# fgvieira/ngsLD

Hardware: AMD Instinct MI355X
Metric: SNP-pair EM-LD computations/sec @ n_ind=500 (higher is better)
Workload: dtype f64

## Files before the change

include/ngsld.h:

```cpp
#ifndef NGSLD_H
#define NGSLD_H

#include <stddef.h>
#include <stdint.h>

#ifdef __cplusplus
extern "C" {
#endif

typedef struct ngsld_ctx ngsld_ctx;

enum {
  NGSLD_OK = 0,
  NGSLD_ERR_INVALID = -1,
  NGSLD_ERR_DEVICE = -2,
  NGSLD_ERR_NOMEM = -3,
  NGSLD_ERR_NAN = -4,
  NGSLD_ERR_MAF_RANGE = -5,
  NGSLD_ERR_SINK = -6,
  NGSLD_ERR_UNSUPPORTED = -7
};

typedef struct {
  uint64_t max_kb_dist;
// ... 19 lines not shown
  uint32_t n_iter;
} ngsld_rec_ext;

typedef struct {
  uint32_t s1, s2_begin, count, reserved;
  uint64_t mask;
  uint64_t first_record;
} ngsld_item;

typedef struct {
  uint64_t s1_begin, s1_end;
  uint64_t n_pairs;
  uint64_t n_items;
  const ngsld_item *items;
  const ngsld_rec_std *std;
  const ngsld_rec_ext *ext;
  const char *text;
  uint64_t text_len;
} ngsld_batch;

typedef int (*ngsld_sink_fn)(void *user, const ngsld_batch *batch);

typedef int (*ngsld_read_sites_fn)(void *user, uint64_t site_begin, uint64_t n_sites, double *dst);

const char *ngsld_version(void);

int ngsld_create(int device, ngsld_ctx **ctx);
void ngsld_destroy(ngsld_ctx *ctx);
const char *ngsld_last_error(const ngsld_ctx *ctx);

int ngsld_set_geno_raw(ngsld_ctx *ctx, const double *gl_raw, uint64_t n_sites, uint64_t n_ind, int log_scale,
                       int ignore_miss_data, int on_device);
typedef struct {
  int32_t log_scale;
  int32_t ignore_miss_data;
  int32_t on_device;
  int32_t text_semantics;
  int32_t call_geno;
  int32_t per_individual_only;
  double N_thresh;
  double call_thresh;
} ngsld_geno_opts;
int ngsld_set_geno_raw_opts(ngsld_ctx *ctx, const double *gl_raw, uint64_t n_sites, uint64_t n_ind,
                            const ngsld_geno_opts *opts);
int ngsld_set_geno_lkl(ngsld_ctx *ctx, const double *geno_lkl, const double *maf, uint64_t n_sites, uint64_t n_ind,
                       int on_device);
int ngsld_get_maf(ngsld_ctx *ctx, double *maf_out);
int ngsld_set_pos_dist(ngsld_ctx *ctx, const double *pos_dist);

int ngsld_plan(ngsld_ctx *ctx, const ngsld_params *params, uint64_t *n_pairs);
int ngsld_plan_rows(ngsld_ctx *ctx, const uint64_t **row_off, const uint32_t **row_end);

int ngsld_run(ngsld_ctx *ctx, uint64_t s1_begin, uint64_t s1_end, ngsld_sink_fn sink, void *user);

int ngsld_set_text_output(ngsld_ctx *ctx, const char *const *labels, int enable);

int ngsld_reserve_text_buffers(ngsld_ctx *ctx, uint64_t bytes_per_row);

int ngsld_set_replay_source(ngsld_ctx *ctx, ngsld_read_sites_fn read, void *user);
int ngsld_set_replay_matrix(ngsld_ctx *ctx, const double *values);
int ngsld_set_replay(ngsld_ctx *ctx, int enable);
int ngsld_replay_stats(ngsld_ctx *ctx, uint64_t *pairs, uint64_t *sites);

int ngsld_set_exact_store(ngsld_ctx *ctx, int mode);
typedef struct {
  uint64_t pairs_flagged;
  uint64_t pairs_replayed;
  uint64_t pairs_on_device;
  uint64_t pairs_on_host;
  uint64_t sites_reevaluated;
  int32_t exact_store;
  int32_t text_rows_patched;
  double exact_store_build_s;
  uint64_t sites_degenerate;
} ngsld_replay_stats_t;
int ngsld_replay_info(ngsld_ctx *ctx, ngsld_replay_stats_t *out);

int ngsld_run_device(ngsld_ctx *ctx, uint64_t s1_begin, uint64_t s1_end, void *d_std, void *d_ext, void *hip_stream);
int ngsld_finish_device(ngsld_ctx *ctx);

int ngsld_last_kernel_time(ngsld_ctx *ctx, double *total_ms, uint64_t *n_launches, uint64_t *n_pairs);

const char *ngsld_pair_kernel(const ngsld_ctx *ctx);
int ngsld_describe_dispatch(uint64_t n_ind, int ignore_miss_data, char *buf, size_t buf_len);

int ngsld_set_tuning(ngsld_ctx *ctx, uint32_t pairs_per_item, uint64_t batch_pairs);

int ngsld_selftest(ngsld_ctx *ctx);

int ngsld_selftest_format(ngsld_ctx *ctx, uint64_t n, const ngsld_rec_std *std, const ngsld_rec_ext *ext, const double *dist,
                          const double *maf1, const double *maf2, char *text, uint64_t text_cap, uint64_t *row_len,
                          int32_t *needs_host);
int ngsld_selftest_printed(ngsld_ctx *ctx, uint64_t n, const double *x, int32_t precision, int32_t weight_type,
                           double min_weight, int64_t *micro, int32_t *micro_ok, int64_t *label, int32_t *label_rc);

typedef struct {
  uint64_t row_begin, row_end;
  uint64_t site_end;
} ngsld_slab;

int ngsld_window_ends(const double *pos_dist, uint64_t n_sites, const ngsld_params *params, uint32_t *row_end);

int ngsld_plan_slabs(const double *pos_dist, uint64_t n_sites, const ngsld_params *params, uint64_t max_slab_sites,
                     ngsld_slab *slabs, uint64_t cap, uint64_t *n_slabs);

uint64_t ngsld_slab_sites_for_budget(uint64_t n_ind, uint64_t budget_bytes);
uint64_t ngsld_sites_for_budget(uint64_t n_ind, uint64_t budget_bytes, int matrix_copies);

int ngsld_streamed_replay_info(ngsld_replay_stats_t *out);

int ngsld_set_memory_budget(int device, uint64_t bytes);

int ngsld_device_memory(int device, uint64_t *free_bytes, uint64_t *total_bytes);


int ngsld_run_streamed(int device, uint64_t n_sites, uint64_t n_ind, const double *pos_dist,
                       const ngsld_params *params, const ngsld_geno_opts *opts, uint64_t max_slab_sites,
                       ngsld_read_sites_fn read, void *read_user, double *maf_out, ngsld_sink_fn sink,
                       void *sink_user, uint64_t *n_pairs, uint64_t *n_slabs, char *err, size_t errlen);

int ngsld_run_streamed_text(int device, uint64_t n_sites, uint64_t n_ind, const double *pos_dist,
                            const ngsld_params *params, const ngsld_geno_opts *opts, uint64_t max_slab_sites,
                            ngsld_read_sites_fn read, void *read_user, double *maf_out, ngsld_sink_fn sink,
                            void *sink_user, uint64_t *n_pairs, uint64_t *n_slabs, char *err, size_t errlen,
                            const char *const *labels, int text_output);


int ngsld_plan_parts(const double *pos_dist, uint64_t n_sites, const ngsld_params *params, int n_parts, ngsld_slab *parts);

typedef int (*ngsld_multi_sink_fn)(void *user, int part, const ngsld_batch *batch);

int ngsld_run_multi(const int *devices, int n_devices, uint64_t n_sites, uint64_t n_ind, const double *pos_dist,
                    const ngsld_params *params, const ngsld_geno_opts *opts, const double *gl_raw,
                    ngsld_read_sites_fn read, void *read_user, double *maf_out, ngsld_multi_sink_fn sink, void *sink_user,
                    const char *const *labels, int text_output, uint64_t *pairs_per_part, char *err, size_t errlen);

enum { NGSLD_DIST_NONE = 0, NGSLD_DIST_UPLOAD = 1, NGSLD_DIST_PEER_COPY = 2, NGSLD_DIST_RCCL = 3 };
int ngsld_multi_last_distribution(void);

int ngsld_rccl_selftest(int device, uint64_t bytes, char *err, size_t errlen);

typedef struct {
  uint32_t struct_size;
  int32_t field;
  double max_kb_dist;
  double min_weight;
  int32_t weight_type;
  int32_t keep_heavy;
  int32_t precision;
  int32_t reserved;
  const char *const *subset;
  uint64_t n_subset;
} ngsld_prune_params;

typedef struct {
  uint32_t struct_size;
  uint32_t reserved;
  uint64_t pairs;
  uint64_t nodes, edges;
  uint64_t kept, excluded;
  uint64_t rounds;
  uint64_t host_nodes, host_edges, host_steps;
  double pairs_ms, edges_ms, graph_ms, rounds_ms, host_ms, total_ms;
} ngsld_prune_stats;

int ngsld_prune(ngsld_ctx *ctx, const ngsld_prune_params *params, const char *const *labels, uint8_t *site_state,
// ... 75 lines not shown
```

ngsld_amd/capi.py:

```python
from __future__ import annotations

import ctypes as C
import os
import subprocess

import numpy as np

PKG_DIR = os.path.dirname(os.path.abspath(__file__))
REPO_DIR = os.path.dirname(PKG_DIR)
LIB_PATH = os.environ.get("NGSLD_LIB") or os.path.join(PKG_DIR, "libngsld.so")
CLI_PATH = os.path.join(PKG_DIR, "bin", "ngsLD")

OK, ERR_INVALID, ERR_DEVICE, ERR_NOMEM, ERR_NAN, ERR_MAF_RANGE, ERR_SINK, ERR_UNSUPPORTED = 0, -1, -2, -3, -4, -5, -6, -7


class Params(C.Structure):
    _fields_ = [("max_kb_dist", C.c_uint64), ("max_snp_dist", C.c_uint64), ("min_maf", C.c_double),
                ("ignore_miss_data", C.c_int32), ("extend_out", C.c_int32), ("rnd_sample", C.c_double),
                ("seed", C.c_uint64), ("first_row", C.c_uint64)]


class GenoOpts(C.Structure):
    _fields_ = [("log_scale", C.c_int32), ("ignore_miss_data", C.c_int32), ("on_device", C.c_int32),
                ("text_semantics", C.c_int32), ("call_geno", C.c_int32), ("per_individual_only", C.c_int32),
                ("N_thresh", C.c_double), ("call_thresh", C.c_double)]


REC_STD = np.dtype([("r2_ExpG", "<f8"), ("D", "<f8"), ("Dp", "<f8"), ("r2", "<f8")])
REC_EXT = np.dtype([("hap", "<f8", (4,)), ("n_ind_data", "<u4"), ("n_iter", "<u4")])


ITEM = np.dtype([("s1", "<u4"), ("s2_begin", "<u4"), ("count", "<u4"), ("reserved", "<u4"), ("mask", "<u8"),
                 ("first_record", "<u8")])


class Batch(C.Structure):
    _fields_ = [("s1_begin", C.c_uint64), ("s1_end", C.c_uint64), ("n_pairs", C.c_uint64), ("n_items", C.c_uint64),
                ("items", C.c_void_p), ("std", C.c_void_p), ("ext", C.c_void_p), ("text", C.c_void_p),
                ("text_len", C.c_uint64)]


def items_to_pairs(items: np.ndarray) -> tuple[np.ndarray, np.ndarray]:
    if len(items) == 0:
        return np.zeros(0, dtype=np.uint64), np.zeros(0, dtype=np.uint64)
    bits = (items["mask"][:, None] >> np.arange(64, dtype=np.uint64)[None, :]) & np.uint64(1)
    bits &= (np.arange(64)[None, :] < items["count"][:, None]).astype(np.uint64)
    idx, c = np.nonzero(bits)
    return items["s1"][idx].astype(np.uint64), (items["s2_begin"][idx].astype(np.uint64) + c.astype(np.uint64))


def items_from_pairs(s1: np.ndarray, s2: np.ndarray, span: int = 64) -> np.ndarray:
    s1, s2 = np.asarray(s1, dtype=np.int64), np.asarray(s2, dtype=np.int64)
    chunk = (s2 - s1 - 1) // span
    key = s1 * (1 << 32) + chunk
    uniq, first, inv = np.unique(key, return_index=True, return_inverse=True)
    items = np.zeros(len(uniq), dtype=ITEM)
    items["s1"] = s1[first]
    items["s2_begin"] = s1[first] + 1 + chunk[first] * span
    items["first_record"] = first
    np.bitwise_or.at(items["mask"], inv, np.uint64(1) << (s2 - items["s2_begin"][inv]).astype(np.uint64))
    last = np.zeros(len(uniq), dtype=np.int64)
    np.maximum.at(last, inv, s2 - items["s2_begin"][inv].astype(np.int64))
    items["count"] = last + 1
    return items


SINK_FN = C.CFUNCTYPE(C.c_int, C.c_void_p, C.POINTER(Batch))
MULTI_SINK_FN = C.CFUNCTYPE(C.c_int, C.c_void_p, C.c_int, C.POINTER(Batch))
READ_FN = C.CFUNCTYPE(C.c_int, C.c_void_p, C.c_uint64, C.c_uint64, C.c_void_p)
SLAB = np.dtype([("row_begin", "<u8"), ("row_end", "<u8"), ("site_end", "<u8")])

SYMBOLS = [
    "ngsld_version", "ngsld_create", "ngsld_destroy", "ngsld_last_error", "ngsld_set_geno_raw",
    "ngsld_set_geno_raw_opts", "ngsld_set_geno_lkl",
    "ngsld_get_maf", "ngsld_set_pos_dist", "ngsld_plan", "ngsld_plan_rows", "ngsld_run", "ngsld_run_device", "ngsld_set_text_output",
    "ngsld_set_replay_source", "ngsld_set_replay_matrix", "ngsld_set_replay", "ngsld_replay_stats", "ngsld_finish_device",
    "ngsld_set_exact_store", "ngsld_replay_info",
    "ngsld_plan_parts", "ngsld_run_multi", "ngsld_multi_last_distribution", "ngsld_rccl_selftest",
    "ngsld_last_kernel_time", "ngsld_pair_kernel", "ngsld_describe_dispatch", "ngsld_set_tuning", "ngsld_selftest", "ngsld_selftest_format",
    "ngsld_selftest_printed", "ngsld_reserve_text_buffers",
    "ngsld_window_ends", "ngsld_plan_slabs", "ngsld_slab_sites_for_budget", "ngsld_sites_for_budget", "ngsld_streamed_replay_info", "ngsld_set_memory_budget", "ngsld_device_memory", "ngsld_run_streamed", "ngsld_run_streamed_text",
    "ngsld_host_read_geno_bin_range",
    "ngsld_host_set_threads", "ngsld_host_read_pos", "ngsld_host_pos_dist", "ngsld_host_label", "ngsld_host_free_pos", "ngsld_host_pos_slice",
    "ngsld_host_geno_size_ok", "ngsld_host_read_geno_bin", "ngsld_host_read_geno_text", "ngsld_host_format_header", "ngsld_host_format_pair",
    "ngsld_host_format_double", "ngsld_host_write_batch", "ngsld_host_replay_pair", "ngsld_host_missing_call_log",
    "ngsld_host_gz_open", "ngsld_host_gz_close",
    "ngsld_prune", "ngsld_host_prune_graph", "ngsld_host_prune_label",
    "ngsld_decay", "ngsld_decay_bins", "ngsld_host_decay_fit",
    "ngsld_blocks", "ngsld_blocks_sites", "ngsld_blocks_matrix", "ngsld_blocks_text",
    "ngsld_site_ld", "ngsld_site_ld_get",
]


class ReplayStats(C.Structure):
    _fields_ = [("pairs_flagged", C.c_uint64), ("pairs_replayed", C.c_uint64), ("pairs_on_device", C.c_uint64),
                ("pairs_on_host", C.c_uint64), ("sites_reevaluated", C.c_uint64), ("exact_store", C.c_int32),
                ("text_rows_patched", C.c_int32), ("exact_store_build_s", C.c_double), ("sites_degenerate", C.c_uint64)]


class PruneParams(C.Structure):
    _fields_ = [("struct_size", C.c_uint32), ("field", C.c_int32), ("max_kb_dist", C.c_double), ("min_weight", C.c_double),
                ("weight_type", C.c_int32), ("keep_heavy", C.c_int32), ("precision", C.c_int32), ("reserved", C.c_int32),
                ("subset", C.POINTER(C.c_char_p)), ("n_subset", C.c_uint64)]


class PruneStats(C.Structure):
    _fields_ = [("struct_size", C.c_uint32), ("reserved", C.c_uint32), ("pairs", C.c_uint64), ("nodes", C.c_uint64),
                ("edges", C.c_uint64), ("kept", C.c_uint64), ("excluded", C.c_uint64), ("rounds", C.c_uint64),
                ("host_nodes", C.c_uint64), ("host_edges", C.c_uint64), ("host_steps", C.c_uint64),
                ("pairs_ms", C.c_double), ("edges_ms", C.c_double), ("graph_ms", C.c_double), ("rounds_ms", C.c_double),
                ("host_ms", C.c_double), ("total_ms", C.c_double)]


class DecayParams(C.Structure):
    _fields_ = [("struct_size", C.c_uint32), ("fields", C.c_uint32), ("bin_size", C.c_double), ("max_kb_dist", C.c_double),
                ("min_maf", C.c_double)]


class DecayStats(C.Structure):
    _fields_ = [("struct_size", C.c_uint32), ("lds", C.c_uint32), ("pairs", C.c_uint64), ("pairs_counted", C.c_uint64),
                ("bins", C.c_uint64), ("bin_slots", C.c_uint64), ("chunks", C.c_uint64), ("pairs_ms", C.c_double),
                ("bin_ms", C.c_double), ("total_ms", C.c_double)]


class BlocksParams(C.Structure):
    _fields_ = [("struct_size", C.c_uint32), ("fields", C.c_uint32), ("chr", C.c_char_p), ("start", C.c_uint64),
                ("end", C.c_uint64)]


class BlocksStats(C.Structure):
    _fields_ = [("struct_size", C.c_uint32), ("reserved", C.c_uint32), ("members", C.c_uint64), ("sites", C.c_uint64),
                ("pairs", C.c_uint64), ("pairs_in_region", C.c_uint64), ("cells_na", C.c_uint64), ("host_rows", C.c_uint64),
                ("chunks", C.c_uint64), ("pairs_ms", C.c_double), ("scatter_ms", C.c_double), ("format_ms", C.c_double),
                ("total_ms", C.c_double)]


class SiteLdParams(C.Structure):
    _fields_ = [("struct_size", C.c_uint32), ("fields", C.c_uint32), ("max_kb_dist", C.c_double), ("min_maf", C.c_double),
                ("linked_min", C.c_double), ("abs_value", C.c_int32), ("reserved", C.c_int32)]


class SiteLdStats(C.Structure):
    _fields_ = [("struct_size", C.c_uint32), ("lds", C.c_uint32), ("pairs", C.c_uint64), ("pairs_counted", C.c_uint64),
                ("sites_with_pairs", C.c_uint64), ("chunks", C.c_uint64), ("pairs_ms", C.c_double), ("site_ms", C.c_double),
                ("total_ms", C.c_double)]


TEXT_FN = C.CFUNCTYPE(C.c_int, C.c_void_p, C.c_void_p, C.c_uint64)


class DecayFitResult(C.Structure):
    _fields_ = [("rate", C.c_double), ("ld_max", C.c_double), ("ld_min", C.c_double), ("sse", C.c_double),
                ("n_bins", C.c_uint64)]


DECAY_FIELDS = ("r2_ExpG", "D", "Dp", "r2")


class NgsldError(RuntimeError):
    def __init__(self, code: int, msg: str):
        super().__init__(f"ngsld error {code}: {msg}")
        self.code = code
        self.msg = msg


def build(force: bool = False, jobs: int = 8) -> None:
    csrc = os.path.join(PKG_DIR, "csrc")
    if force:
        subprocess.check_call(["make", "-s", "-C", csrc, "clean"])
    subprocess.check_call(["make", "-s", f"-j{jobs}", "-C", csrc, "all"])


_lib = None


def lib() -> C.CDLL:
    global _lib
    if _lib is None:
        if not os.path.exists(LIB_PATH):
            raise FileNotFoundError(f"{LIB_PATH} is missing: run ngsld_amd.capi.build() (or make -C ngsld_amd/csrc); "
                                    "there is no fallback implementation")
        L = C.CDLL(LIB_PATH)
        vp, u64, dbl = C.c_void_p, C.c_uint64, C.c_double
        L.ngsld_version.restype = C.c_char_p
        L.ngsld_create.argtypes = [C.c_int, C.POINTER(vp)]
        L.ngsld_destroy.argtypes = [vp]
        L.ngsld_destroy.restype = None
        L.ngsld_last_error.argtypes = [vp]
        L.ngsld_last_error.restype = C.c_char_p
        L.ngsld_set_geno_raw.argtypes = [vp, vp, u64, u64, C.c_int, C.c_int, C.c_int]
        L.ngsld_set_geno_raw_opts.argtypes = [vp, vp, u64, u64, C.POINTER(GenoOpts)]
        L.ngsld_set_geno_lkl.argtypes = [vp, vp, vp, u64, u64, C.c_int]
        L.ngsld_get_maf.argtypes = [vp, vp]
        L.ngsld_set_pos_dist.argtypes = [vp, vp]
        L.ngsld_plan.argtypes = [vp, C.POINTER(Params), C.POINTER(u64)]
        L.ngsld_plan_rows.argtypes = [vp, C.POINTER(C.POINTER(C.c_uint64)), C.POINTER(C.POINTER(C.c_uint32))]
        L.ngsld_run.argtypes = [vp, u64, u64, SINK_FN, vp]
        L.ngsld_run_device.argtypes = [vp, u64, u64, vp, vp, vp]
        if hasattr(L, "ngsld_set_replay_source"):
            L.ngsld_set_replay_source.argtypes = [vp, READ_FN, vp]
            if hasattr(L, "ngsld_set_replay_matrix"):
                L.ngsld_set_replay_matrix.argtypes = [vp, vp]
            L.ngsld_set_replay.argtypes = [vp, C.c_int]
            L.ngsld_replay_stats.argtypes = [vp, C.POINTER(u64), C.POINTER(u64)]
        if hasattr(L, "ngsld_replay_info"):
            L.ngsld_set_exact_store.argtypes = [vp, C.c_int]
            L.ngsld_replay_info.argtypes = [vp, C.POINTER(ReplayStats)]
            L.ngsld_finish_device.argtypes = [vp]
        if hasattr(L, "ngsld_set_text_output"):
            L.ngsld_set_text_output.argtypes = [vp, C.POINTER(C.c_char_p), C.c_int]
        L.ngsld_last_kernel_time.argtypes = [vp, C.POINTER(dbl), C.POINTER(u64), C.POINTER(u64)]
        L.ngsld_set_tuning.argtypes = [vp, C.c_uint32, u64]
        if hasattr(L, "ngsld_pair_kernel"):
            L.ngsld_pair_kernel.argtypes = [vp]
            L.ngsld_pair_kernel.restype = C.c_char_p
        L.ngsld_selftest.argtypes = [vp]
        if hasattr(L, "ngsld_selftest_format"):
            L.ngsld_selftest_format.argtypes = [vp, u64, vp, vp, vp, vp, vp, C.c_char_p, u64, vp, C.POINTER(C.c_int32)]
            L.ngsld_selftest_printed.argtypes = [vp, u64, vp, C.c_int32, C.c_int32, dbl, vp, vp, vp, vp]
        L.ngsld_window_ends.argtypes = [vp, u64, C.POINTER(Params), vp]
        L.ngsld_plan_slabs.argtypes = [vp, u64, C.POINTER(Params), u64, vp, u64, C.POINTER(u64)]
        L.ngsld_slab_sites_for_budget.argtypes = [u64, u64]
        L.ngsld_slab_sites_for_budget.restype = u64
        if hasattr(L, "ngsld_sites_for_budget"):
            L.ngsld_sites_for_budget.argtypes = [u64, u64, C.c_int]
            L.ngsld_sites_for_budget.restype = u64
        L.ngsld_device_memory.argtypes = [C.c_int, C.POINTER(u64), C.POINTER(u64)]
        L.ngsld_run_streamed.argtypes = [C.c_int, u64, u64, vp, C.POINTER(Params), C.POINTER(GenoOpts), u64, READ_FN, vp,
                                         vp, SINK_FN, vp, C.POINTER(u64), C.POINTER(u64), C.c_char_p, C.c_size_t]
        if hasattr(L, "ngsld_run_multi"):
            L.ngsld_plan_parts.argtypes = [vp, u64, C.POINTER(Params), C.c_int, vp]
            L.ngsld_run_multi.argtypes = [C.POINTER(C.c_int), C.c_int, u64, u64, vp, C.POINTER(Params), C.POINTER(GenoOpts),
                                          vp, READ_FN, vp, vp, MULTI_SINK_FN, vp, C.POINTER(C.c_char_p), C.c_int,
                                          C.POINTER(u64), C.c_char_p, C.c_size_t]
        if hasattr(L, "ngsld_multi_last_distribution"):
            L.ngsld_multi_last_distribution.argtypes = []
        if hasattr(L, "ngsld_rccl_selftest"):
            L.ngsld_rccl_selftest.argtypes = [C.c_int, u64, C.c_char_p, C.c_size_t]
        L.ngsld_host_read_geno_bin_range.argtypes = [C.c_char_p, u64, u64, u64, vp, C.c_char_p, C.c_size_t]
        L.ngsld_host_set_threads.argtypes = [C.c_int]
        L.ngsld_host_set_threads.restype = None
        L.ngsld_host_read_pos.argtypes = [C.c_char_p, C.c_int, u64, C.POINTER(vp), C.c_char_p, C.c_size_t]
        L.ngsld_host_pos_dist.argtypes = [vp]
        L.ngsld_host_pos_dist.restype = C.POINTER(dbl)
        L.ngsld_host_label.argtypes = [vp, u64]
        L.ngsld_host_label.restype = C.c_char_p
        L.ngsld_host_free_pos.argtypes = [vp]
        L.ngsld_host_free_pos.restype = None
        L.ngsld_host_pos_slice.argtypes = [vp, u64, u64]
        L.ngsld_host_pos_slice.restype = vp
        L.ngsld_host_geno_size_ok.argtypes = [u64, u64, u64]
        L.ngsld_host_read_geno_bin.argtypes = [C.c_char_p, u64, u64, vp, C.c_char_p, C.c_size_t]
        L.ngsld_host_read_geno_text.argtypes = [C.c_char_p, C.c_int, C.c_int, u64, u64, vp, C.POINTER(C.c_int),
                                                C.c_char_p, C.c_size_t]
        L.ngsld_host_format_header.argtypes = [C.c_char_p, C.c_size_t, C.c_int]
        L.ngsld_host_format_header.restype = C.c_size_t
        L.ngsld_host_format_pair.argtypes = [C.c_char_p, C.c_size_t, C.c_char_p, C.c_char_p, dbl, vp, vp, dbl, dbl]
        L.ngsld_host_format_pair.restype = C.c_size_t
        L.ngsld_host_format_double.argtypes = [C.c_char_p, C.c_size_t, dbl, C.c_int]
        L.ngsld_host_format_double.restype = C.c_size_t
        L.ngsld_host_write_batch.argtypes = [C.POINTER(Batch), vp, vp, vp, C.c_int, C.c_int]
        L.ngsld_host_replay_pair.argtypes = [vp, vp, u64, C.POINTER(GenoOpts), vp, vp, vp]
        if hasattr(L, "ngsld_host_gz_open"):
            L.ngsld_host_gz_open.argtypes = [C.c_char_p, C.c_int, C.POINTER(vp), C.POINTER(C.c_int)]
            L.ngsld_host_gz_close.argtypes = [vp]
        if hasattr(L, "ngsld_prune"):
            L.ngsld_prune.argtypes = [vp, C.POINTER(PruneParams), C.POINTER(C.c_char_p), vp, C.POINTER(PruneStats)]
            L.ngsld_host_prune_graph.argtypes = [u64, vp, u64, vp, vp, vp, C.c_int, vp, C.POINTER(u64)]
            L.ngsld_host_prune_label.argtypes = [dbl, C.c_int, C.c_char, C.POINTER(C.c_int64)]
        if hasattr(L, "ngsld_decay"):
            L.ngsld_decay.argtypes = [vp, C.POINTER(DecayParams), C.POINTER(DecayStats)]
            L.ngsld_decay_bins.argtypes = [vp, u64, vp, vp, vp, C.POINTER(u64)]
            L.ngsld_host_decay_fit.argtypes = [u64, vp, vp, C.c_int, dbl, dbl, C.POINTER(DecayFitResult)]
        if hasattr(L, "ngsld_blocks"):
            L.ngsld_blocks.argtypes = [vp, C.POINTER(BlocksParams), C.POINTER(C.c_char_p), C.POINTER(BlocksStats)]
            L.ngsld_blocks_sites.argtypes = [vp, u64, vp, C.POINTER(u64)]
            L.ngsld_blocks_matrix.argtypes = [vp, C.c_int, vp, vp]
            L.ngsld_blocks_text.argtypes = [vp, C.c_int, TEXT_FN, vp, C.POINTER(BlocksStats)]
        if hasattr(L, "ngsld_site_ld"):
            L.ngsld_site_ld.argtypes = [vp, C.POINTER(SiteLdParams), C.POINTER(SiteLdStats)]
            L.ngsld_site_ld_get.argtypes = [vp, C.c_int, vp, vp, vp, vp, vp]
        _lib = L
    return _lib


def prune_label(x: float, prec: int = 4, weight_type: str = "a") -> int | None:
    out = C.c_int64()
    rc = lib().ngsld_host_prune_label(float(x), prec, weight_type.encode(), C.byref(out))
    if rc == ERR_INVALID:
        return None
    if rc != OK:
        raise NgsldError(rc, "label out of range")
    return out.value


# ... 546 lines not shown
                    exts.append(np.frombuffer(C.string_at(b.ext, n * REC_EXT.itemsize), dtype=REC_EXT).copy())
            items = np.frombuffer(C.string_at(b.items, b.n_items * ITEM.itemsize), dtype=ITEM) if b.n_items else \
                np.zeros(0, dtype=ITEM)
            a, bb = items_to_pairs(items)
            assert len(a) == n
            if len(items):
                assert np.array_equal(items["first_record"], np.concatenate([[0], np.cumsum(
                    [bin(int(m)).count("1") for m in items["mask"]])[:-1]]).astype(np.uint64))
            s1s.append(a)
            s2s.append(bb)
            return 0

        cb = SINK_FN(sink)
        self._check(self._L.ngsld_run(self._h, s1_begin, s1_end, cb, None))
        cat = lambda xs, dt: np.concatenate(xs) if xs else np.zeros(0, dtype=dt)
        return (cat(s1s, np.uint64), cat(s2s, np.uint64), cat(stds, REC_STD),
                cat(exts, REC_EXT) if self.extend_out else None)

    def run_to_fd(self, s1_begin: int, s1_end: int, fd: int, pos_handle, pos_dist: np.ndarray | None, maf: np.ndarray,
                  n_threads: int) -> int:
        maf = np.ascontiguousarray(maf, dtype=np.float64)
        pd_ptr = None if pos_dist is None else np.ascontiguousarray(pos_dist, dtype=np.float64).ctypes.data
        total, rc_box = [0], [0]

        libc = C.CDLL(None, use_errno=True)
        libc.write.argtypes = [C.c_int, C.c_void_p, C.c_size_t]
        libc.write.restype = C.c_ssize_t

        def sink(_user, bp):
            b = bp.contents
            total[0] += b.n_pairs
            if b.text:
                off = 0
                while off < b.text_len:
                    w = libc.write(fd, b.text + off, min(b.text_len - off, 1 << 30))
                    if w <= 0:
                        return 1
                    off += w
                return 0
            rc_box[0] = self._L.ngsld_host_write_batch(bp, pos_handle, pd_ptr, maf.ctypes.data, n_threads, fd)
            return 0 if rc_box[0] == OK else 1

        self._check(self._L.ngsld_run(self._h, s1_begin, s1_end, SINK_FN(sink), None))
        return total[0]

    def set_text_output(self, labels: list[str] | None, enable: bool = True) -> None:
        arr = None
        if labels is not None:
            arr = (C.c_char_p * len(labels))(*[l.encode() for l in labels])
        self._check(self._L.ngsld_set_text_output(self._h, arr, int(enable)))

    def run_text(self, s1_begin: int = 0, s1_end: int | None = None) -> tuple[bytes, int]:
        s1_end = self.n_sites if s1_end is None else s1_end
        parts, fallbacks = [], [0]

        def sink(_user, bp):
            b = bp.contents
            if b.text:
                parts.append(C.string_at(b.text, b.text_len))
            else:
                fallbacks[0] += 1
            return 0

        self._check(self._L.ngsld_run(self._h, s1_begin, s1_end, SINK_FN(sink), None))
        return b"".join(parts), fallbacks[0]

    def run_discard(self, s1_begin: int = 0, s1_end: int | None = None) -> int:
        s1_end = self.n_sites if s1_end is None else s1_end
        total = [0]

        def sink(_user, bp):
            total[0] += bp.contents.n_pairs
            return 0

        self._check(self._L.ngsld_run(self._h, s1_begin, s1_end, SINK_FN(sink), None))
        return total[0]

    def run_device(self, s1_begin: int, s1_end: int, d_std: int, d_ext: int | None, stream: int | None = None) -> None:
        self._check(self._L.ngsld_run_device(self._h, s1_begin, s1_end, d_std, d_ext, stream))

    def pair_kernel(self) -> str:
        return self._L.ngsld_pair_kernel(self._h).decode()

    def last_kernel_time(self) -> tuple[float, int, int]:
        ms, nl, npairs = C.c_double(), C.c_uint64(), C.c_uint64()
        self._check(self._L.ngsld_last_kernel_time(self._h, C.byref(ms), C.byref(nl), C.byref(npairs)))
        return ms.value, nl.value, npairs.value

    def prune(self, labels: list[str] | None, field: int = 7, max_kb_dist: float = float("inf"), min_weight: float = 0.0,
              weight_type: str = "a", keep_heavy: bool = False, subset: list[str] | None = None,
              precision: int = 4) -> tuple[np.ndarray, dict]:
        arr = None if labels is None else (C.c_char_p * len(labels))(*[l.encode() for l in labels])
        sub = None if subset is None else (C.c_char_p * max(len(subset), 1))(*[l.encode() for l in subset])
        p = PruneParams(C.sizeof(PruneParams), field, float(max_kb_dist), float(min_weight), ord(weight_type), int(keep_heavy),
                        precision, 0, sub, 0 if subset is None else len(subset))
        st = PruneStats()
        st.struct_size = C.sizeof(PruneStats)
        state = np.zeros(max(self.n_sites, 1), dtype=np.uint8)
        self._check(self._L.ngsld_prune(self._h, C.byref(p), arr, state.ctypes.data, C.byref(st)))
        return state[:self.n_sites], {k: getattr(st, k) for k, _ in PruneStats._fields_ if k not in ("struct_size", "reserved")}

    def decay(self, ld=("r2",), bin_size: float = 250, max_kb_dist: float = float("inf"),
              min_maf: float = 0.0) -> tuple[dict, dict]:
        ld = (ld,) if isinstance(ld, str) else tuple(ld)
        bad = [f for f in ld if f not in DECAY_FIELDS]
        if bad or not ld:
            raise ValueError(f"ld must name some of {DECAY_FIELDS}: {bad}")
        mask = sum(1 << DECAY_FIELDS.index(f) for f in set(ld))
        names = [f for k, f in enumerate(DECAY_FIELDS) if (mask >> k) & 1]
        p = DecayParams(C.sizeof(DecayParams), mask, float(bin_size), float(max_kb_dist), float(min_maf))
        st = DecayStats()
        st.struct_size = C.sizeof(DecayStats)
        self._check(self._L.ngsld_decay(self._h, C.byref(p), C.byref(st)))
        nb = st.bins
        dist = np.zeros(max(nb, 1))
        cnt = np.zeros(max(nb, 1), dtype=np.uint64)
        mean = np.zeros((max(nb, 1), len(names)))
        got = C.c_uint64()
        self._check(self._L.ngsld_decay_bins(self._h, nb, dist.ctypes.data, cnt.ctypes.data, mean.ctypes.data, C.byref(got)))
        assert got.value == nb
        bins = {"dist": dist[:nb], "n": cnt[:nb]}
        for k, f in enumerate(names):
            bins[f] = mean[:nb, k].copy()
        return bins, {k: getattr(st, k) for k, _ in DecayStats._fields_ if k != "struct_size"}

    def site_ld(self, ld=("r2",), max_kb_dist: float = float("inf"), min_maf: float = 0.0, linked_min: float = 0.5,
                abs_value: bool = True) -> tuple[dict, dict]:
        ld = (ld,) if isinstance(ld, str) else tuple(ld)
        bad = [f for f in ld if f not in DECAY_FIELDS]
        if bad or not ld:
            raise ValueError(f"ld must name some of {DECAY_FIELDS}: {bad}")
        mask = sum(1 << DECAY_FIELDS.index(f) for f in set(ld))
        p = SiteLdParams(C.sizeof(SiteLdParams), mask, float(max_kb_dist), float(min_maf), float(linked_min), int(bool(abs_value)), 0)
        st = SiteLdStats()
        st.struct_size = C.sizeof(SiteLdStats)
        self._check(self._L.ngsld_site_ld(self._h, C.byref(p), C.byref(st)))
        m = max(self.n_sites, 1)
        sites = {"n": np.zeros(m, dtype=np.uint64)}
        for k, f in enumerate(DECAY_FIELDS):
            if not (mask >> k) & 1:
                continue
            sites[f"sum_{f}"], sites[f"max_{f}"] = np.zeros(m, dtype=np.int64), np.zeros(m, dtype=np.int64)
            sites[f"linked_{f}"], sites[f"mean_{f}"] = np.zeros(m, dtype=np.uint64), np.zeros(m)
            self._check(self._L.ngsld_site_ld_get(self._h, 4 + k, sites["n"].ctypes.data, sites[f"sum_{f}"].ctypes.data,
                                                  sites[f"max_{f}"].ctypes.data, sites[f"linked_{f}"].ctypes.data,
                                                  sites[f"mean_{f}"].ctypes.data))
        sites = {k: v[:self.n_sites] for k, v in sites.items()}
        return sites, {k: getattr(st, k) for k, _ in SiteLdStats._fields_ if k != "struct_size"}

    def blocks(self, labels: list[str], chr: str, start: int, end: int,
               ld=("r2", "Dp")) -> tuple[np.ndarray, dict, dict]:
        ld = (ld,) if isinstance(ld, str) else tuple(ld)
        bad = [f for f in ld if f not in DECAY_FIELDS]
        if bad or not ld:
            raise ValueError(f"ld must name some of {DECAY_FIELDS}: {bad}")
        mask = sum(1 << DECAY_FIELDS.index(f) for f in set(ld))
        arr = (C.c_char_p * max(len(labels), 1))(*[l.encode() for l in labels]) if labels is not None else None
        p = BlocksParams(C.sizeof(BlocksParams), mask, chr.encode(), int(start), int(end))
        st = BlocksStats()
        st.struct_size = C.sizeof(BlocksStats)
        self._check(self._L.ngsld_blocks(self._h, C.byref(p), arr, C.byref(st)))
        m = st.sites
        sites = np.zeros(max(m, 1), dtype=np.uint64)
        got = C.c_uint64()
        self._check(self._L.ngsld_blocks_sites(self._h, m, sites.ctypes.data, C.byref(got)))
        assert got.value == m
# ... 26 lines not shown
```

ngsld_amd/csrc/cli_main.cpp:

```cpp
#include <getopt.h>
#include <zlib.h>
#include <sys/stat.h>
#include <sys/mman.h>
#include <unistd.h>

#include <cmath>
#include <cstdio>
#include <cstdlib>
#include <cstring>
#include <ctime>
#include <memory>
#include <string>
#include <algorithm>
#include <chrono>
#include <thread>
#include <vector>

#include "../../include/ngsld.h"
#include "../../include/ngsld_host.h"
#include "knobs.h"
#include "host_buf.h"

namespace {

// ... 1096 lines not shown
    if (site_begin + n > r->n_sites) return 1;
    memcpy(dst, r->raw + site_begin * r->n_ind * 3, n * r->n_ind * 3 * sizeof(double));
    return 0;
  };
  if (ngsld::test_knob_is("REPLAY_SOURCE", "0"))
    raw.reset();
  else if (ngsld::test_knob_is("REPLAY_SOURCE", "callback")) {
    if (ngsld_set_replay_source(ctx, read_raw, &raw_src) != NGSLD_OK) error("ngsld_set_replay_source", ngsld_last_error(ctx));
  } else if (ngsld_set_replay_matrix(ctx, raw.get()) != NGSLD_OK)
    error("ngsld_set_replay_matrix", ngsld_last_error(ctx));

  if (pars.verbose >= 1) fprintf(stderr, "==> Getting sites coordinates\n");
  ngsld_pos *pos = nullptr;
  if (pars.in_pos) {
    if (early.pos_done) {
      if (early.pos_rc != NGSLD_OK) error(pos_error_function(early.pos_err, pars.in_pos), early.pos_err);
      pos = early.pos;
    } else if (ngsld_host_read_pos(pars.in_pos, pars.in_pos_header ? 1 : 0, pars.n_sites, &pos, err, sizeof(err)) != NGSLD_OK)
      error(pos_error_function(err, pars.in_pos), err);
    if (pars.verbose >= 6)
      for (uint64_t s = 0; s < (pars.n_sites < 10 ? pars.n_sites : 10); s++)
        fprintf(stderr, "%lu\t%f\n", (unsigned long)s, ngsld_host_pos_dist(pos)[s]);
  }
  if (ngsld_set_pos_dist(ctx, pos ? ngsld_host_pos_dist(pos) : nullptr) != NGSLD_OK)
    error("ngsld_set_pos_dist", ngsld_last_error(ctx));

  if (pars.verbose >= 1) fprintf(stderr, "==> Launching threads...\n");
  ngsld_params lp;
  lp.max_kb_dist = pars.max_kb_dist;
  lp.max_snp_dist = pars.max_snp_dist;
  lp.min_maf = pars.min_maf;
  lp.ignore_miss_data = pars.ignore_miss_data ? 1 : 0;
  lp.extend_out = pars.extend_out ? 1 : 0;
  lp.rnd_sample = pars.rnd_sample;
  lp.seed = pars.seed;
  lp.first_row = 0;
  uint64_t n_pairs = 0;
  timing_report.mark("positions");
  if (ngsld_plan(ctx, &lp, &n_pairs) != NGSLD_OK) error("ngsld_plan", ngsld_last_error(ctx));
  std::vector<double> maf(pars.n_sites);
  if (ngsld_get_maf(ctx, maf.data()) != NGSLD_OK) error("ngsld_get_maf", ngsld_last_error(ctx));
  timing_report.mark("plan");
  if (write_tsv && !host_text_only()) {
    std::vector<const char *> lab;
    if (pos) {
      lab.resize(pars.n_sites);
      for (uint64_t s = 0; s < pars.n_sites; s++) lab[s] = ngsld_host_label(pos, s);
    }
    if (ngsld_set_text_output(ctx, pos ? lab.data() : nullptr, 1) != NGSLD_OK)
      error("ngsld_set_text_output", ngsld_last_error(ctx));
  }
  if (pars.verbose >= 1) fprintf(stderr, "==> Waiting for all threads to finish...\n");
  SinkState sink;
  sink.pars = &pars;
  sink.pos = pos;
  sink.pos_dist = pos ? ngsld_host_pos_dist(pos) : nullptr;
  sink.maf = &maf;
  timing_report.mark("labels to the device");
  rc = write_tsv ? ngsld_run(ctx, 0, pars.n_sites, write_batch, &sink) : NGSLD_OK;
  timing_report.mark("pair kernels + text + write");
  if (rc == NGSLD_ERR_MAF_RANGE) error("haplo_freq", ngsld_last_error(ctx));
  if (rc != NGSLD_OK) error("ngsld_run", ngsld_last_error(ctx));
  if (prune.given) {
    run_prune(ctx, pars, prune, pos);
    timing_report.mark("pruning");
  }
  if (decay.given) {
    run_decay(ctx, pars, decay);
    timing_report.mark("LD decay");
  }
  if (blocks.given) {
    run_blocks(ctx, pars, blocks, pos);
    timing_report.mark("LD blocks");
  }
  if (site.given) {
    run_site(ctx, pars, site, pos);
    timing_report.mark("site LD");
  }
  if (write_tsv && pars.verbose >= 2) {
    ngsld_replay_stats_t st{};
    (void)ngsld_replay_info(ctx, &st);
    fprintf(stderr, "==> %lu of %lu pairs replayed in the reference's operation order (%lu on the device, %lu on host threads)\n",
            (unsigned long)st.pairs_replayed, (unsigned long)n_pairs, (unsigned long)st.pairs_on_device, (unsigned long)st.pairs_on_host);
  }

  if (pars.verbose >= 1) fprintf(stderr, "==> Freeing memory...\n");
  close_output(pars.out_fh);
  ngsld_host_free_pos(pos);
  ngsld_destroy(ctx);
  timing_report.mark("free");
  if (pars.verbose >= 1) fprintf(stderr, "Done!\n");
  return 0;
}
```

ngsld_amd/csrc/engine.h:

```cpp
#pragma once

#include "knobs.h"

#include <hip/hip_runtime.h>
#include <sched.h>
#include <dlfcn.h>
#include <sys/mman.h>

#include <algorithm>
#include <atomic>
#include <chrono>
#include <cmath>
#include <condition_variable>
#include <functional>
#include <cstdio>
#include <cstdlib>
#include <cstring>
#include <limits>
#include <mutex>
#include <new>
#include <string>
#include <thread>
#include <unordered_map>
#include <vector>
// ... 141 lines not shown
    while ((int)threads_.size() < T - 1) {
      const int id = (int)threads_.size() + 1;
      threads_.emplace_back([this, id] { loop(id); });
    }
    {
      std::lock_guard<std::mutex> lk(mu_);
      job_ = [&fn](int t) { fn(t); };
      n_ = T;
      left_ = T - 1;
      ++epoch_;
    }
    cv_.notify_all();
    fn(0);
    std::unique_lock<std::mutex> lk(mu_);
    done_.wait(lk, [this] { return left_ == 0; });
    job_ = nullptr;
  }

 private:
  void loop(int id) {
    uint64_t seen = 0;
    for (;;) {
      std::function<void(int)> job;
      {
        std::unique_lock<std::mutex> lk(mu_);
        cv_.wait(lk, [&] { return stop_ || epoch_ != seen; });
        if (stop_) return;
        seen = epoch_;
        if (id >= n_) continue;
        job = job_;
      }
      job(id);
      std::lock_guard<std::mutex> lk(mu_);
      if (--left_ == 0) done_.notify_all();
    }
  }
  std::vector<std::thread> threads_;
  std::mutex mu_;
  std::condition_variable cv_, done_;
  std::function<void(int)> job_;
  int n_ = 0, left_ = 0;
  uint64_t epoch_ = 0;
  bool stop_ = false;
};

}
}

using namespace ngsld;
using namespace ngsld::eng;

struct FlagRow {
  uint64_t rec, off;
  uint32_t len, s1, s2, pad;
};
constexpr uint32_t kFlagRowsCap = 1024;

struct ngsld_ctx {
  int device = 0;
  hipStream_t stream = nullptr, stream2 = nullptr, copy_stream = nullptr;
  hipStream_t text_stream = nullptr;
  hipEvent_t ev_scan_done[3] = {nullptr, nullptr, nullptr};
  std::string err;

  uint64_t n_sites = 0, n_ind = 0;
  uint32_t np = 0;
  PairConfig cfg{};
  bool have_geno = false;
  DevBuf<double> d_planes, d_maf, d_mean, d_rsx, d_sc4;
  DevBuf<int> d_status;
  std::vector<double> h_maf, h_pos_dist;
  DevBuf<uint64_t> d_hard_masks;
  DevBuf<double> d_hard_u;
  DevBuf<int> d_all_hard, d_odd_missing;
  int h_odd_missing = 0;
  bool missing_canonical = false;
  int h_all_hard = 0, h_prep_status = 0;
  uint32_t mask_words = 0;
  DevBuf<uint8_t> d_skip;
  DevBuf<uint32_t> d_skip_count;
  uint32_t h_skip_count = 0;
  bool skip_on = true;
  bool skip_kernels = false;

  bool planned = false;
  ngsld_params params{};
  std::vector<uint64_t> h_row_off, h_item_off;
  std::vector<uint32_t> h_row_end;
  std::vector<uint8_t> h_keep;
  std::vector<Item> h_items;
  std::vector<uint64_t> h_run_off;
  uint64_t run_len = 0;
  std::vector<uint64_t> run_ends;
  int n_cus = 256;
  DevBuf<Run> d_runs;
  DevBuf<uint64_t> d_row_off, d_item_off, d_row_seed, d_row_count;
  DevBuf<uint32_t> d_row_end;
  DevBuf<uint8_t> d_keep;
  DevBuf<Item> d_items;
  uint64_t n_items = 0;

  int kernel_choice = kChooseAuto;
  uint32_t pairs_per_item = 16;
  uint64_t batch_pairs = 1ull << 23;
  bool batch_pairs_set = false;

  static constexpr int kSlots = 3;
  DevBuf<ngsld_rec_std> d_std[kSlots];
  DevBuf<ngsld_rec_ext> d_ext[kSlots];
  PinBuf<ngsld_rec_std> h_std[kSlots];
  PinBuf<ngsld_rec_ext> h_ext[kSlots];
  hipEvent_t ev_kernel_done[kSlots] = {nullptr, nullptr, nullptr}, ev_copy_done[kSlots] = {nullptr, nullptr, nullptr};
  bool run_direct = true, run_taper = true;
  int run_streams = 1;
  bool timed_overlap = false;

  bool text_mode = false, have_labels = false;
  uint64_t max_label = 6;
  DevBuf<char> d_labels, d_text[kSlots], d_scan_tmp, d_scan_tmp_b;
  DevBuf<uint64_t> d_label_off, d_lens[kSlots], d_offs[kSlots], d_text_meta[kSlots];
  DevBuf<double> d_cum;
  DevBuf<uint32_t> d_infc;
  PinBuf<char> h_text[kSlots];
  PinBuf<uint64_t> h_text_meta[kSlots];
  std::thread reserve_thread;

  bool replay_on = true;
  ngsld_read_sites_fn replay_read = nullptr;
  void *replay_user = nullptr;
  const double *replay_matrix = nullptr;
  std::mutex replay_mu;
  hipStream_t replay_stream = nullptr;
  std::mutex replay_stream_mu;
  ngsld_geno_opts gopts{};
  bool normalised = false;
  DevBuf<uint32_t> d_flags[kSlots], d_flags_dev;
  PinBuf<uint32_t> h_flags[kSlots], h_flags_dev;
  PinBuf<uint32_t> h_flag_bits;
  PinBuf<FlagRow> h_flag_rows[kSlots];
  uint32_t flag_cap[kSlots] = {0, 0, 0}, flag_cap_dev = 0;
  bool replay_device = true;
  uint64_t replayed_on_device = 0;
  uint64_t text_rows_patched = 0;
  DevBuf<double> d_xplanes, d_xmaf;
  DevBuf<double> d_xT;
  std::atomic<bool> xT_ready{false};
  DevBuf<uint32_t> d_xperm;
  DevBuf<uint32_t> d_xdepth;
  struct LaneScratch {
    DevBuf<ReplayEntry> list;
    DevBuf<uint64_t> keys_a, keys_b;
    DevBuf<uint32_t> vals_a, vals_b;
    DevBuf<char> temp;
    void release() { list.release(); keys_a.release(); keys_b.release(); vals_a.release(); vals_b.release(); temp.release(); }
  } lane_scratch[kSlots], lane_scratch_dev;
  PinBuf<double> h_xstage[2];
  std::thread exact_thread;
  std::atomic<int> exact_state{0};
  std::atomic<uint64_t> exact_frontier{0};
  std::atomic<bool> exact_cancel{false};
  std::mutex exact_mu;
  std::condition_variable exact_cv;
  int exact_rc = 0;
  std::string exact_msg;
  hipStream_t exact_stream = nullptr;
  ReplayPool exact_pool;
// ... 145 lines not shown
  EventPair() = default;
  EventPair(const EventPair &) = delete;
  EventPair &operator=(const EventPair &) = delete;
  ~EventPair() {
    if (a) (void)hipEventDestroy(a);
    if (b) (void)hipEventDestroy(b);
  }
  hipError_t create() {
    hipError_t e = hipEventCreate(&a);
    return e == hipSuccess ? hipEventCreate(&b) : e;
  }
  hipError_t add_elapsed(double *ms) const {
    float t = 0.f;
    const hipError_t e = hipEventElapsedTime(&t, a, b);
    if (e == hipSuccess) *ms += t;
    return e;
  }
};

int launch_record_items(ngsld_ctx *c, EventPair &ev, uint64_t r0, uint64_t r1, double *ms, uint64_t *chunks,
                        const std::function<void(const ngsld_item *items, uint64_t n_items)> &launch);

inline unsigned blocks_for(uint64_t threads, unsigned per_block = 256) { return (unsigned)((threads + per_block - 1) / per_block); }
inline double ms_since(std::chrono::steady_clock::time_point t0) {
  return std::chrono::duration<double, std::milli>(std::chrono::steady_clock::now() - t0).count();
}
template <class P, class S>
int check_struct_sizes(ngsld_ctx *c, const P *p, const char *p_name, const S *stats, const char *s_name) {
  if (p == nullptr || p->struct_size != sizeof(P))
    return fail(c, NGSLD_ERR_INVALID, std::string(p_name) + ": struct_size must be sizeof(" + p_name + ")");
  if (stats != nullptr && stats->struct_size < sizeof(uint32_t)) return fail(c, NGSLD_ERR_INVALID, std::string(s_name) + ": struct_size not set");
  return NGSLD_OK;
}
template <class S>
void copy_stats(S *out, const S &s) {
  if (out == nullptr) return;
  const uint32_t want = out->struct_size;
  std::memcpy(out, &s, std::min<size_t>(want, sizeof(S)));
  out->struct_size = want;
}
inline int field_list(uint32_t mask, int field[4]) {
  int ns = 0;
  for (int f = 0; f < 4; ++f)
    if ((mask >> f) & 1u) field[ns++] = f;
  return ns;
}

int send_flag_rows(ngsld_ctx *c, const uint32_t *d_flags, uint32_t cap, bool dev_applied, const uint64_t *d_offs, const uint64_t *d_lens,
                   uint64_t n_records, uint64_t base, FlagRow *h_rows, hipStream_t st);
int replay_pairs_on_host(ngsld_ctx *c, const uint32_t *s1, const uint32_t *s2, size_t n, ngsld_rec_std *out_std, ngsld_rec_ext *out_ext);
unsigned usable_threads();
hipStream_t replay_stream_of(ngsld_ctx *c);
int ensure_host_items(ngsld_ctx *c);
int fetch_replay_site(ngsld_ctx *c, uint64_t s, std::vector<double> &tmp, ReplaySite *out);
int flagged_records(ngsld_ctx *c, const uint32_t *h_head, const uint32_t *d_flags, uint32_t cap, uint64_t n,
                    std::vector<uint64_t> &recs, bool dev_applied = false);
bool room_for(uint64_t need_bytes, uint64_t device_margin, uint64_t budget_margin);
bool lkl_device_eligible(const ngsld_ctx *c);
bool exact_store_is_free(const ngsld_ctx *c);
inline bool exact_store_started(const ngsld_ctx *c) { return c->exact_state.load() >= 1; }
int start_exact_store(ngsld_ctx *c);
int reserve_device_run(ngsld_ctx *c, uint64_t n_records);
int wait_exact_store(ngsld_ctx *c, uint64_t need_sites, bool *have);
int ensure_exact_store(ngsld_ctx *c);
void stop_exact_store(ngsld_ctx *c);
inline uint64_t exact_sites_needed(const ngsld_ctx *c, uint64_t r0, uint64_t r1) {
  uint64_t need = r1;
  for (uint64_t r = r0; r < r1 && r < c->h_row_end.size(); ++r) need = std::max<uint64_t>(need, c->h_row_end[r]);
  return std::min<uint64_t>(need, c->n_sites);
}
bool exact_store_wanted(const ngsld_ctx *c, uint64_t pending);
int try_device_replay_lkl(ngsld_ctx *c, uint32_t *d_flags, uint32_t cap, uint64_t out_base, uint64_t n, ngsld_rec_std *d_std,
                          ngsld_rec_ext *d_ext, hipStream_t st, bool flag_text, int slot, bool *applied, uint64_t need_sites);
int device_replay_lkl(ngsld_ctx *c, uint32_t *d_flags, uint32_t cap, uint64_t out_base, uint64_t n, ngsld_rec_std *d_std,
                      ngsld_rec_ext *d_ext, hipStream_t st, bool flag_text, int slot);
int replay_flagged(ngsld_ctx *c, const std::vector<uint64_t> &recs, uint64_t base, ngsld_rec_std *h_std,
                   ngsld_rec_ext *h_ext, ngsld_rec_std *d_std, ngsld_rec_ext *d_ext, hipStream_t st,
                   std::vector<uint32_t> *sites1 = nullptr, std::vector<uint32_t> *sites2 = nullptr);
int reset_flags(ngsld_ctx *c, DevBuf<uint32_t> &buf, uint64_t n, uint32_t cap, hipStream_t stream);
int send_flag_head(ngsld_ctx *c, const uint32_t *d_flags, uint32_t *h_head, uint32_t cap, hipStream_t st, bool with_list = true);
int device_replay(ngsld_ctx *c, uint32_t *d_flags, uint32_t cap, uint64_t out_base, uint64_t n, ngsld_rec_std *d_std,
                  ngsld_rec_ext *d_ext, hipStream_t st, int slot);
int finish_device_run(ngsld_ctx *c);

}
}
```

ngsld_amd/csrc/engine.hip:

```cpp
#include "engine.h"

#include <atomic>

namespace ngsld {
namespace eng {

thread_local std::string g_create_error;

int set_geno_common(ngsld_ctx *c, const double *gl, const double *maf, uint64_t n_sites, uint64_t n_ind,
                    const ngsld_geno_opts &o, bool normalised) {
  if (c == nullptr) return NGSLD_ERR_INVALID;
  const int log_scale = o.log_scale, ignore_miss = o.ignore_miss_data, on_device = o.on_device;
  Range range_("ngsld:set_geno (upload + per-site prep)");
  if (o.call_geno && o.N_thresh > o.call_thresh)
    return fail(c, NGSLD_ERR_INVALID, "missing data threshold must be smaller than calling genotype threshold!");
  if (gl == nullptr || n_sites == 0 || n_ind == 0) return fail(c, NGSLD_ERR_INVALID, "empty genotype matrix");
  if (normalised && maf == nullptr) return fail(c, NGSLD_ERR_INVALID, "maf missing");
  if (n_sites >= 0xffffffffull) return fail(c, NGSLD_ERR_UNSUPPORTED, "n_sites must be below 2^32 - 1");
  PairConfig cfg;
  if (!pair_config(n_ind, &cfg, c->kernel_choice, ignore_miss != 0))
    return fail(c, NGSLD_ERR_UNSUPPORTED, "n_ind is outside the supported range");
  HIP_TRY(c, hipSetDevice(c->device));
  (void)hipGetLastError();
  {
// ... 58 lines not shown
    const char *pe = test_knob("PREP_EXACT");
    a.exact_chain = (pe != nullptr && std::strcmp(pe, "0") != 0) ? 1 : 0;
  }
  a.N_thresh = o.N_thresh;
  a.call_thresh = o.call_thresh;
  a.maf = c->d_maf.p;
  a.mean_e = c->d_mean.p;
  a.rsx = c->d_rsx.p;
  a.status = c->d_status.p;
  c->missing_canonical = false;
  const bool look_for_odd_missing = o.text_semantics && log_scale && !o.call_geno && !normalised;
  if (look_for_odd_missing) {
    HIP_TRY(c, c->d_odd_missing.resize(1));
    HIP_TRY(c, hipMemsetAsync(c->d_odd_missing.p, 0, sizeof(int), c->stream));
    a.odd_missing = c->d_odd_missing.p;
    a.missing_canon = replay_missing_raw_text();
  }
  if (on_device) {
    a.raw = gl;
    a.maf_in = maf;
    a.site0 = 0;
    a.n_sites = n_sites;
    HIP_TRY(c, launch_prep(a, c->stream));
  } else {
    const uint64_t site_bytes = n_ind * 3 * sizeof(double);
    uint64_t stage_bytes = 64ull << 20;
    if (const char *e = test_knob("STAGE_BYTES")) stage_bytes = std::strtoull(e, nullptr, 10);
    uint64_t chunk = stage_bytes / site_bytes;
    if (chunk < 1) chunk = 1;
    if (chunk > n_sites) chunk = n_sites;
    DevBuf<double> stage[2], maf_stage[2];
    hipEvent_t prepped[2] = {nullptr, nullptr};
    for (int k = 0; k < 2; ++k) {
      HIP_TRY(c, stage[k].resize(chunk * n_ind * 3));
      if (normalised) HIP_TRY(c, maf_stage[k].resize(chunk));
      HIP_TRY(c, hipEventCreateWithFlags(&prepped[k], hipEventDisableTiming));
    }
    int rc = NGSLD_OK;
    uint64_t k = 0;
    if (trace) std::fprintf(stderr, "[trace] set_geno: device buffers + staging allocated at %.2f ms\n", ms_since());
    for (uint64_t s0 = 0; s0 < n_sites && rc == NGSLD_OK; s0 += chunk, ++k) {
      const int b = (int)(k & 1);
      const uint64_t m = std::min(chunk, n_sites - s0);
      hipError_t e = hipSuccess;
      if (k >= 2) e = hipEventSynchronize(prepped[b]);
      if (e == hipSuccess)
        e = hipMemcpyAsync(stage[b].p, gl + s0 * n_ind * 3, m * site_bytes, hipMemcpyHostToDevice, c->copy_stream);
      if (e == hipSuccess && normalised)
        e = hipMemcpyAsync(maf_stage[b].p, maf + s0, m * sizeof(double), hipMemcpyHostToDevice, c->copy_stream);
      if (e == hipSuccess) e = hipStreamSynchronize(c->copy_stream);
      if (trace) std::fprintf(stderr, "[trace] set_geno: chunk %llu (%llu sites) on the device at %.2f ms\n", (unsigned long long)k, (unsigned long long)m, ms_since());
      a.raw = stage[b].p;
      a.maf_in = normalised ? maf_stage[b].p : nullptr;
      a.site0 = s0;
      a.n_sites = m;
      if (e == hipSuccess) e = launch_prep(a, c->stream);
      if (e == hipSuccess) e = hipEventRecord(prepped[b], c->stream);
      if (e != hipSuccess) rc = hip_fail(c, e, "chunked genotype upload");
    }
    hipError_t e = hipStreamSynchronize(c->stream);
    if (trace) std::fprintf(stderr, "[trace] set_geno: last prep kernel done at %.2f ms\n", ms_since());
    for (int q = 0; q < 2; ++q) {
      stage[q].release();
      maf_stage[q].release();
      if (prepped[q]) (void)hipEventDestroy(prepped[q]);
    }
    if (trace) std::fprintf(stderr, "[trace] set_geno: staging buffers freed at %.2f ms\n", ms_since());
    if (rc != NGSLD_OK) return rc;
    if (e != hipSuccess) return hip_fail(c, e, "chunked genotype upload");
  }
  c->h_skip_count = 0;
  const bool look_for_skip = c->skip_on && c->replay_on && c->replay_device && c->exact_mode != 0;
  c->skip_kernels = cfg.kernel == kRun || (cfg.kernel == kMulti && cfg.form == 0 && cfg.waves == 2);
  if (look_for_skip) {
    HIP_TRY(c, c->d_skip.resize(n_sites));
    HIP_TRY(c, c->d_skip_count.resize(1));
    HIP_TRY(c, hipMemsetAsync(c->d_skip_count.p, 0, sizeof(uint32_t), c->stream));
    HIP_TRY(c, launch_site_skip(c->d_planes.p, 3ull * c->np, c->np, (uint32_t)n_ind, ignore_miss, c->d_maf.p, n_sites, c->d_skip.p,
                                c->d_skip_count.p, c->stream));
    HIP_TRY(c, hipMemcpyAsync(&c->h_skip_count, c->d_skip_count.p, sizeof(uint32_t), hipMemcpyDeviceToHost, c->stream));
  } else {
    c->d_skip.release();
  }
  HIP_TRY(c, launch_pack_scalars(c->d_maf.p, c->d_mean.p, c->d_rsx.p, c->d_skip.p, c->d_sc4.p, n_sites, c->stream));
  int &all_hard = c->h_all_hard;
  all_hard = 0;
  const char *hk = test_knob("HARD_KERNEL");
  const bool try_hard = n_ind <= kHardMaxInd && !o.per_individual_only && !(hk != nullptr && std::strcmp(hk, "0") == 0);
  if (try_hard) {
    c->mask_words = (uint32_t)((n_ind + 63) / 64);
    HIP_TRY(c, c->d_hard_masks.resize((size_t)n_sites * 4 * c->mask_words));
    HIP_TRY(c, c->d_hard_u.resize(n_sites));
    HIP_TRY(c, c->d_all_hard.resize(1));
    all_hard = 1;
    HIP_TRY(c, hipMemcpyAsync(c->d_all_hard.p, &all_hard, sizeof(int), hipMemcpyHostToDevice, c->stream));
    HIP_TRY(c, launch_classify_hard(c->d_planes.p, 3ull * c->np, c->np, (uint32_t)n_ind, n_sites, c->d_hard_masks.p,
                                    c->d_hard_u.p, c->d_all_hard.p, c->stream));
    HIP_TRY(c, hipMemcpyAsync(&all_hard, c->d_all_hard.p, sizeof(int), hipMemcpyDeviceToHost, c->stream));
    if (trace) std::fprintf(stderr, "[trace] set_geno: called-genotype check enqueued at %.2f ms\n", ms_since());
  }
  c->h_maf.resize(n_sites);
  int &status = c->h_prep_status;
  status = 0;
  HIP_TRY(c, hipMemcpyAsync(c->h_maf.data(), c->d_maf.p, n_sites * sizeof(double), hipMemcpyDeviceToHost, c->stream));
  HIP_TRY(c, hipMemcpyAsync(&status, c->d_status.p, sizeof(int), hipMemcpyDeviceToHost, c->stream));
  c->h_odd_missing = 1;
  if (look_for_odd_missing)
    HIP_TRY(c, hipMemcpyAsync(&c->h_odd_missing, c->d_odd_missing.p, sizeof(int), hipMemcpyDeviceToHost, c->stream));
  HIP_TRY(c, hipStreamSynchronize(c->stream));
  c->missing_canonical = look_for_odd_missing && c->h_odd_missing == 0;
  if (trace) std::fprintf(stderr, "[trace] set_geno: scalars packed, called-genotype check, maf on the host at %.2f ms\n", ms_since());
  if (status == NGSLD_ERR_NAN) return fail(c, NGSLD_ERR_NAN, "NaN found! Is the file format correct?");
  if (try_hard && all_hard) {
    c->cfg.kernel = kHard;
    c->cfg.group = 16;
    c->cfg.slots = 1;
    c->cfg.waves = 1;
  } else {
    c->d_hard_masks.release();
    c->d_hard_u.release();
  }
  c->have_geno = true;
  return NGSLD_OK;
}
}
}

extern "C" {

const char *ngsld_version(void) { return "ngsld-amd 0.9.0 (gfx950; reference ngsLD 1.2.1)"; }

int ngsld_create(int device, ngsld_ctx **out) {
  if (out == nullptr) return NGSLD_ERR_INVALID;
  *out = nullptr;
  int n_dev = 0;
  hipError_t e = hipGetDeviceCount(&n_dev);
  if (e != hipSuccess || n_dev == 0) {
    g_create_error = std::string("no HIP device available (") + hipGetErrorString(e) +
                     "); this library has no CPU fallback";
    return NGSLD_ERR_DEVICE;
  }
  if (device < 0 || device >= n_dev) {
    g_create_error = "device index out of range";
    return NGSLD_ERR_INVALID;
  }
  hipDeviceProp_t prop;
  e = hipGetDeviceProperties(&prop, device);
  if (e != hipSuccess) {
    g_create_error = std::string("hipGetDeviceProperties: ") + hipGetErrorString(e);
    return NGSLD_ERR_DEVICE;
  }
  if (std::strncmp(prop.gcnArchName, "gfx950", 6) != 0) {
    g_create_error = std::string("device is ") + prop.gcnArchName + ", this build targets gfx950 (MI355X) only";
    return NGSLD_ERR_DEVICE;
  }
  ngsld_ctx *c = new (std::nothrow) ngsld_ctx();
  if (c == nullptr) return NGSLD_ERR_NOMEM;
  c->device = device;
  if (prop.multiProcessorCount > 0) c->n_cus = prop.multiProcessorCount;
  if (const char *k = std::getenv("NGSLD_PAIR_KERNEL")) {
    c->kernel_choice = std::strcmp(k, "multi") == 0 ? kChooseMulti
                       : (std::strcmp(k, "ab") == 0 ? kChooseAB
                          : (std::strcmp(k, "stream") == 0 ? kChoosePlainStream : (std::strcmp(k, "abm") == 0 ? kChooseABMulti
                                                               : (std::strcmp(k, "bres") == 0 ? kChooseResidentStream : kChooseAuto))));
  }
  if (const char *k = test_knob("BATCH_PAIRS")) {
    const uint64_t v = std::strtoull(k, nullptr, 10);
    if (v > 0) {
      c->batch_pairs = v;
      c->batch_pairs_set = true;
    }
  }
  if (const char *k = std::getenv("NGSLD_REPLAY")) c->replay_on = std::strcmp(k, "0") != 0;
  if (const char *k = std::getenv("NGSLD_REPLAY_THREADS")) c->replay_threads = std::atoi(k);
  if (const char *k = std::getenv("NGSLD_REPLAY_DEVICE")) c->replay_device = std::strcmp(k, "0") != 0;
  if (const char *k = std::getenv("NGSLD_REPLAY_SKIP")) c->skip_on = std::strcmp(k, "0") != 0;
  if (const char *k = std::getenv("NGSLD_EXACT_STORE")) c->exact_mode = std::max(0, std::min(2, std::atoi(k)));
  if (const char *k = test_knob("RUN_DIRECT")) c->run_direct = std::strcmp(k, "0") != 0;
  if (const char *k = test_knob("RUN_TAPER")) c->run_taper = std::strcmp(k, "0") != 0;
  if (const char *k = test_knob("RUN_STREAMS")) c->run_streams = std::atoi(k) >= 2 ? 2 : 1;
  if ((e = hipSetDevice(device)) != hipSuccess || (e = hipStreamCreate(&c->stream)) != hipSuccess ||
      (e = hipStreamCreate(&c->stream2)) != hipSuccess || (e = hipStreamCreate(&c->copy_stream)) != hipSuccess) {
    g_create_error = std::string("stream setup: ") + hipGetErrorString(e);
    delete c;
    return NGSLD_ERR_DEVICE;
  }
  for (int k = 0; k < ngsld_ctx::kSlots; ++k) {
    (void)hipEventCreateWithFlags(&c->ev_kernel_done[k], hipEventDisableTiming);
    (void)hipEventCreateWithFlags(&c->ev_copy_done[k], hipEventDisableTiming);
  }
  *out = c;
  return NGSLD_OK;
}

void ngsld_destroy(ngsld_ctx *c) {
  if (c == nullptr) return;
  if (c->reserve_thread.joinable()) c->reserve_thread.join();
  stop_exact_store(c);
  (void)hipSetDevice(c->device);
  (void)hipDeviceSynchronize();
  if (c->exact_stream) (void)hipStreamDestroy(c->exact_stream);
  c->d_planes.release(); c->d_maf.release(); c->d_mean.release(); c->d_rsx.release(); c->d_sc4.release(); c->d_runs.release(); c->d_skip.release(); c->d_skip_count.release();
  c->d_hard_masks.release(); c->d_hard_u.release(); c->d_all_hard.release();
  c->d_xplanes.release(); c->d_xmaf.release(); c->d_xT.release(); c->d_xdepth.release(); c->d_xperm.release(); c->h_xstage[0].release(); c->h_xstage[1].release();
  c->lane_scratch_dev.release();
  for (int k = 0; k < ngsld_ctx::kSlots; ++k) c->lane_scratch[k].release();
  c->d_labels.release(); c->d_scan_tmp.release(); c->d_scan_tmp_b.release(); c->d_label_off.release(); c->d_cum.release(); c->d_infc.release();
  for (int k = 0; k < ngsld_ctx::kSlots; ++k) {
    c->d_text[k].release(); c->d_lens[k].release(); c->d_offs[k].release(); c->d_text_meta[k].release();
    c->h_text[k].release(); c->h_text_meta[k].release();
  }
  c->d_status.release(); c->d_row_off.release(); c->d_item_off.release(); c->d_row_end.release();
  c->d_row_seed.release(); c->d_row_count.release(); c->d_keep.release(); c->d_items.release();
  for (int k = 0; k < ngsld_ctx::kSlots; ++k) {
    c->d_std[k].release(); c->d_ext[k].release(); c->h_std[k].release(); c->h_ext[k].release();
    if (c->ev_kernel_done[k]) (void)hipEventDestroy(c->ev_kernel_done[k]);
    if (c->ev_copy_done[k]) (void)hipEventDestroy(c->ev_copy_done[k]);
  }
  for (auto &ev : c->ev_pool) {
    (void)hipEventDestroy(ev.first);
    (void)hipEventDestroy(ev.second);
  }
  if (c->stream) (void)hipStreamDestroy(c->stream);
  if (c->stream2) (void)hipStreamDestroy(c->stream2);
  if (c->copy_stream) (void)hipStreamDestroy(c->copy_stream);
  if (c->text_stream) (void)hipStreamDestroy(c->text_stream);
  for (int k = 0; k < 3; ++k)
    if (c->ev_scan_done[k]) (void)hipEventDestroy(c->ev_scan_done[k]);
  if (c->replay_stream) (void)hipStreamDestroy(c->replay_stream);
  delete c;
}

const char *ngsld_last_error(const ngsld_ctx *c) { return c ? c->err.c_str() : g_create_error.c_str(); }

int ngsld_set_geno_raw(ngsld_ctx *c, const double *gl_raw, uint64_t n_sites, uint64_t n_ind, int log_scale,
                       int ignore_miss_data, int on_device) try {
  ngsld_geno_opts o{};
  o.log_scale = log_scale;
  o.ignore_miss_data = ignore_miss_data;
  o.on_device = on_device;
  return set_geno_common(c, gl_raw, nullptr, n_sites, n_ind, o, false);
} NGSLD_CATCH(c)

int ngsld_set_geno_raw_opts(ngsld_ctx *c, const double *gl_raw, uint64_t n_sites, uint64_t n_ind,
                            const ngsld_geno_opts *opts) try {
  if (opts == nullptr) return c ? fail(c, NGSLD_ERR_INVALID, "opts is NULL") : NGSLD_ERR_INVALID;
  return set_geno_common(c, gl_raw, nullptr, n_sites, n_ind, *opts, false);
} NGSLD_CATCH(c)

int ngsld_set_geno_lkl(ngsld_ctx *c, const double *geno_lkl, const double *maf, uint64_t n_sites, uint64_t n_ind,
                       int on_device) try {
  ngsld_geno_opts o{};
  o.on_device = on_device;
  return set_geno_common(c, geno_lkl, maf, n_sites, n_ind, o, true);
} NGSLD_CATCH(c)

int ngsld_get_maf(ngsld_ctx *c, double *maf_out) try {
  if (c == nullptr || maf_out == nullptr) return NGSLD_ERR_INVALID;
  if (!c->have_geno) return fail(c, NGSLD_ERR_INVALID, "no genotype data set");
  std::memcpy(maf_out, c->h_maf.data(), c->n_sites * sizeof(double));
  return NGSLD_OK;
} NGSLD_CATCH(c)

int ngsld_set_pos_dist(ngsld_ctx *c, const double *pos_dist) try {
  if (c == nullptr) return NGSLD_ERR_INVALID;
  if (!c->have_geno) return fail(c, NGSLD_ERR_INVALID, "set the genotype data before the positions");
  c->planned = false;
  c->clear_blocks();
  if (pos_dist == nullptr)
    c->h_pos_dist.assign(c->n_sites, std::numeric_limits<double>::infinity());
  else
    c->h_pos_dist.assign(pos_dist, pos_dist + c->n_sites);
  return NGSLD_OK;
} NGSLD_CATCH(c)
const char *ngsld_pair_kernel(const ngsld_ctx *c) {
  if (c == nullptr || !c->have_geno) return "";
  switch (effective_kernel(c->cfg, c->params.ignore_miss_data != 0)) {
    case kGroup: return "group";
    case kMulti: return c->cfg.form == 1 ? "multi-ab" : "multi";
    case kStream: return "stream";
    case kRun: return "run";
    case kHard: return "hard";
    case kRunAB: return "ab";
    default: return "";
  }
}

int ngsld_describe_dispatch(uint64_t n_ind, int ignore_miss_data, char *buf, size_t buf_len) {
  if (buf == nullptr || buf_len == 0) return NGSLD_ERR_INVALID;
  buf[0] = 0;
  PairConfig cfg;
  const bool masked = ignore_miss_data != 0;
  if (!pair_config(n_ind, &cfg, kChooseAuto, masked)) return NGSLD_ERR_UNSUPPORTED;
  const char *family = "";
  int slots = cfg.slots, waves = cfg.waves;
  switch (effective_kernel(cfg, masked)) {
    case kGroup: family = "group"; break;
    case kMulti:
      family = cfg.form == 1 ? "multi-ab" : "multi";
      if (cfg.form == 0) multi_shape(cfg, masked, &slots, &waves);
      break;
    case kStream: family = "stream"; break;
    case kRun: family = "run"; break;
    case kRunAB: family = "ab"; break;
    default: return NGSLD_ERR_UNSUPPORTED;
  }
  const int n = std::snprintf(buf, buf_len, "%s %dx%d lanes=%d np=%u", family, waves, slots, cfg.group, cfg.np);
  return (n < 0 || (size_t)n >= buf_len) ? NGSLD_ERR_INVALID : NGSLD_OK;
}

int ngsld_set_tuning(ngsld_ctx *c, uint32_t pairs_per_item, uint64_t batch_pairs) {
  if (c == nullptr) return NGSLD_ERR_INVALID;
  c->clear_blocks();
  if (pairs_per_item) {
    c->pairs_per_item = pairs_per_item;
    c->planned = false;
  }
  if (batch_pairs) {
    c->batch_pairs = batch_pairs;
    c->batch_pairs_set = true;
  }
  return NGSLD_OK;
}

int ngsld_selftest(ngsld_ctx *c) try {
  if (c == nullptr) return NGSLD_ERR_INVALID;
  HIP_TRY(c, hipSetDevice(c->device));
  (void)hipGetLastError();
  std::vector<double> in(320), out(71, 0.0);
  uint64_t st = 0x9E3779B97F4A7C15ull;
  for (auto &v : in) {
    st = st * 6364136223846793005ull + 1442695040888963407ull;
    v = (double)(st >> 11) / 9007199254740992.0 + 1e-3;
  }
  for (int l = 0; l < 64; ++l) in[256 + l] *= std::pow(10.0, -(l % 30));
  DevBuf<double> d_in, d_out;
  HIP_TRY(c, d_in.resize(in.size()));
  HIP_TRY(c, d_out.resize(out.size()));
  HIP_TRY(c, hipMemcpy(d_in.p, in.data(), in.size() * sizeof(double), hipMemcpyHostToDevice));
  HIP_TRY(c, launch_selftest(d_in.p, d_out.p, c->stream));
  HIP_TRY(c, hipStreamSynchronize(c->stream));
  HIP_TRY(c, hipMemcpy(out.data(), d_out.p, out.size() * sizeof(double), hipMemcpyDeviceToHost));
  d_in.release();
  d_out.release();
  for (int k = 0; k < 7; ++k) {
    const int v = k < 4 ? k : k - 4;
    const double got = k < 4 ? out[k] : out[68 + v];
    long double ref = 0;
    for (int l = 0; l < 64; ++l) ref += in[v * 64 + l];
    if (!(std::fabs((double)(got - ref)) <= 1e-14 * std::fabs((double)ref))) {
      char buf[160];
      std::snprintf(buf, sizeof(buf), "%s value %d: got %.17g expected %.17Lg", k < 4 ? "wave_sum4" : "wave_sum3", v, got, ref);
      return fail(c, NGSLD_ERR_DEVICE, buf);
    }
  }
  for (int l = 0; l < 64; ++l) {
    const double ref = 1.0 / in[256 + l];
    if (std::fabs(out[4 + l] - ref) > 4.5e-16 * ref) {
      char buf[160];
      std::snprintf(buf, sizeof(buf), "rcp_refined lane %d: got %.17g expected %.17g", l, out[4 + l], ref);
      return fail(c, NGSLD_ERR_DEVICE, buf);
    }
  }
  return NGSLD_OK;
} NGSLD_CATCH(c)

int ngsld_selftest_format(ngsld_ctx *c, uint64_t n, const ngsld_rec_std *std_rec, const ngsld_rec_ext *ext_rec, const double *dist,
                          const double *maf1, const double *maf2, char *text, uint64_t text_cap, uint64_t *row_len,
// ... 143 lines not shown
```

ngsld_amd/csrc/engine_plan.hip:

```cpp
#include "engine.h"

namespace ngsld {
namespace eng {

void plan_rows(const std::vector<double> &pos_dist, const std::vector<double> &maf, const ngsld_params &p,
               uint64_t n, std::vector<uint32_t> &row_end) {
  row_end.assign(n, 0);
  const bool use_dist = p.max_kb_dist > 0;
  const double limit = (double)(p.max_kb_dist * 1000);
  bool exact = true;
  std::vector<double> cum;
  std::vector<uint32_t> seg;
  if (use_dist) {
    cum.assign(n, 0.0);
    seg.assign(n, 0);
    double run = 0.0;
    uint32_t sg = 0;
    for (uint64_t s = 0; s < n; ++s) {
      const double g = pos_dist[s];
      if (std::isinf(g) && g > 0) {
        if (s > 0) ++sg;
      } else if (s > 0) {
        if (!(g >= 1.0) || g != std::floor(g) || run + g > 9.0e15) exact = false;
        run += g;
// ... 34 lines not shown
  const uint64_t n = c->n_sites;
  uint64_t tail_len = std::max<uint64_t>(1, run_len / 8);
  uint64_t tail_pairs = (uint64_t)c->n_cus * run_len * item_span(c->cfg, c->pairs_per_item);
  if (const char *e = test_knob("TAIL_LEN")) tail_len = (uint64_t)std::max(0l, atol(e));
  if (const char *e = test_knob("TAIL_PAIRS")) tail_pairs = std::strtoull(e, nullptr, 10);
  std::vector<uint8_t> in_tail(n, 0);
  if (tail_len > 0 && tail_len < run_len) {
    uint64_t begin = 0;
    for (const uint64_t end : launch_ends) {
      if (end > n || end < begin) continue;
      for (uint64_t s1 = end; s1 > begin && c->h_row_off[end] - c->h_row_off[s1 - 1] <= tail_pairs; --s1) in_tail[s1 - 1] = 1;
      begin = end;
    }
  }
  std::vector<Run> runs;
  c->h_run_off.assign(n + 1, 0);
  for (uint64_t s1 = 0; s1 < n; ++s1) {
    const uint64_t i0 = c->h_item_off[s1], m = c->h_item_off[s1 + 1] - i0;
    const uint64_t len = in_tail[s1] ? tail_len : run_len;
    const uint64_t parts = (m + len - 1) / len;
    for (uint64_t q = 0; q < parts; ++q) {
      const uint64_t b = i0 + m * q / parts, e = i0 + m * (q + 1) / parts;
      runs.push_back(Run{(uint32_t)b, (uint32_t)(e - b)});
    }
    c->h_run_off[s1 + 1] = runs.size();
  }
  if (c->run_len != 0) HIP_TRY(c, hipDeviceSynchronize());
  HIP_TRY(c, c->d_runs.resize(runs.empty() ? 1 : runs.size()));
  if (!runs.empty())
    HIP_TRY(c, hipMemcpy(c->d_runs.p, runs.data(), runs.size() * sizeof(Run), hipMemcpyHostToDevice));
  c->run_len = run_len;
  c->run_ends = launch_ends;
  return NGSLD_OK;
}
}
}

extern "C" {

int ngsld_plan(ngsld_ctx *c, const ngsld_params *p, uint64_t *n_pairs) try {
  if (c == nullptr || p == nullptr) return NGSLD_ERR_INVALID;
  if (!c->have_geno) return fail(c, NGSLD_ERR_INVALID, "no genotype data set");
  if (c->h_pos_dist.size() != c->n_sites) {
    if (p->max_kb_dist > 0)
      return fail(c, NGSLD_ERR_INVALID, "position file necessary in order to filter by maximum distance!");
    c->h_pos_dist.assign(c->n_sites, std::numeric_limits<double>::infinity());
  }
  if (p->min_maf < 0 || p->min_maf > 1)
    return fail(c, NGSLD_ERR_INVALID, "minimum allele frequency must be in [0,1]!");
  HIP_TRY(c, hipSetDevice(c->device));
  (void)hipGetLastError();
  Range range_("ngsld:plan");
  {
    const int rcp = finish_device_run(c);
    if (rcp != NGSLD_OK) return rcp;
  }
  const uint64_t n = c->n_sites;
  c->params = *p;
  c->planned = false;
  c->clear_blocks();
  if (!(p->rnd_sample >= 0 && p->rnd_sample <= 1))
    return fail(c, NGSLD_ERR_INVALID, "proportion of comparisons to sample must be in ]0,1]!");
  const bool sampling = p->rnd_sample > 0 && p->rnd_sample < 1;
  c->replayed_sites = 0;
  if (c->replay_on && (c->replay_read != nullptr || c->replay_matrix != nullptr) && !c->normalised) {
    bool changed = false;
    std::vector<double> tmp;
    ReplaySite site;
    for (uint64_t s = 0; s < n; ++s) {
      const double m = c->h_maf[s], t = std::fabs(m) * 1e6;
      const bool tie = p->min_maf > 0 && std::fabs(m - p->min_maf) <= 1e-12;
      const bool edge = p->extend_out && std::fabs((t - std::floor(t)) - 0.5) < 1e-6;
      if (!tie && !edge) continue;
      const int rcs = fetch_replay_site(c, s, tmp, &site);
      if (rcs != NGSLD_OK) return fail(c, rcs, "the replay source callback failed");
      ++c->replayed_sites;
      if (site.maf != m && !(site.maf != site.maf && m != m)) {
        c->h_maf[s] = site.maf;
        changed = true;
      }
    }
    if (changed) {
      HIP_TRY(c, hipMemcpy(c->d_maf.p, c->h_maf.data(), n * sizeof(double), hipMemcpyHostToDevice));
      HIP_TRY(c, launch_pack_scalars(c->d_maf.p, c->d_mean.p, c->d_rsx.p, c->d_skip.p, c->d_sc4.p, n, c->stream));
    }
  }
  plan_rows(c->h_pos_dist, c->h_maf, *p, n, c->h_row_end);
  c->h_keep.resize(n);
  for (uint64_t s = 0; s < n; ++s) c->h_keep[s] = (c->h_maf[s] < p->min_maf) ? 0 : 1;
  const uint64_t ch = item_span(c->cfg, c->pairs_per_item);
  c->h_item_off.resize(n + 1);
  c->h_item_off[0] = 0;
  for (uint64_t s1 = 0; s1 < n; ++s1) {
    const uint64_t end = c->h_row_end[s1];
    const uint64_t span = end > s1 + 1 ? end - (s1 + 1) : 0;
    c->h_item_off[s1 + 1] = c->h_item_off[s1] + (span + ch - 1) / ch;
  }
  c->n_items = c->h_item_off[n];
  if (uses_runs(c->cfg.kernel)) {
    if (c->n_items > 0xffffffffull) return fail(c, NGSLD_ERR_UNSUPPORTED, "more than 2^32 work items in one plan");
    c->run_len = 0;
  }
  HIP_TRY(c, c->d_row_end.resize(n));
  HIP_TRY(c, c->d_keep.resize(n));
  HIP_TRY(c, c->d_row_off.resize(n + 1));
  HIP_TRY(c, c->d_item_off.resize(n + 1));
  HIP_TRY(c, c->d_row_count.resize(n));
  HIP_TRY(c, c->d_items.resize(c->n_items ? c->n_items : 1));
  HIP_TRY(c, hipMemcpyAsync(c->d_row_end.p, c->h_row_end.data(), n * sizeof(uint32_t), hipMemcpyHostToDevice, c->stream));
  HIP_TRY(c, hipMemcpyAsync(c->d_keep.p, c->h_keep.data(), n, hipMemcpyHostToDevice, c->stream));
  HIP_TRY(c, hipMemcpyAsync(c->d_item_off.p, c->h_item_off.data(), (n + 1) * sizeof(uint64_t), hipMemcpyHostToDevice, c->stream));
  std::vector<uint64_t> seeds;
  if (sampling) {
    seeds.resize(n);
    Taus master;
    master.set(p->seed);
    for (uint64_t k = 0; k < p->first_row; ++k) master.get();
    for (uint64_t s = 0; s < n; ++s) seeds[s] = master.row_seed();
    HIP_TRY(c, c->d_row_seed.resize(n));
    HIP_TRY(c, hipMemcpyAsync(c->d_row_seed.p, seeds.data(), n * sizeof(uint64_t), hipMemcpyHostToDevice, c->stream));
  }
  ItemArgs ia{};
  ia.row_end = c->d_row_end.p;
  ia.keep = c->d_keep.p;
  ia.row_seed = sampling ? c->d_row_seed.p : nullptr;
  ia.row_off = c->d_row_off.p;
  ia.item_off = c->d_item_off.p;
  ia.row_count = c->d_row_count.p;
  ia.items = c->d_items.p;
  ia.n_sites = (uint32_t)n;
  ia.span = (uint32_t)ch;
  ia.rnd_sample = p->rnd_sample;
  ia.count_only = 1;
  HIP_TRY(c, launch_items(ia, c->stream));
  std::vector<uint64_t> counts(n);
  HIP_TRY(c, hipMemcpyAsync(counts.data(), c->d_row_count.p, n * sizeof(uint64_t), hipMemcpyDeviceToHost, c->stream));
  HIP_TRY(c, hipStreamSynchronize(c->stream));
  c->h_row_off.resize(n + 1);
  c->h_row_off[0] = 0;
  for (uint64_t s1 = 0; s1 < n; ++s1) c->h_row_off[s1 + 1] = c->h_row_off[s1] + counts[s1];
  HIP_TRY(c, hipMemcpyAsync(c->d_row_off.p, c->h_row_off.data(), (n + 1) * sizeof(uint64_t), hipMemcpyHostToDevice, c->stream));
  ia.count_only = 0;
  HIP_TRY(c, launch_items(ia, c->stream));
  c->h_items.clear();
  HIP_TRY(c, hipStreamSynchronize(c->stream));
  if (uses_runs(c->cfg.kernel)) {
    const int rcr = build_runs(c, kRunItems, std::vector<uint64_t>{n});
    if (rcr != NGSLD_OK) return rcr;
  }
  c->planned = true;
  if (n_pairs) *n_pairs = c->h_row_off[n];
  return NGSLD_OK;
} NGSLD_CATCH(c)

int ngsld_plan_rows(ngsld_ctx *c, const uint64_t **row_off, const uint32_t **row_end) {
  if (c == nullptr) return NGSLD_ERR_INVALID;
  if (!c->planned) return fail(c, NGSLD_ERR_INVALID, "ngsld_plan has not been called");
  if (row_off) *row_off = c->h_row_off.data();
  if (row_end) *row_end = c->h_row_end.data();
  return NGSLD_OK;
}
int ngsld_window_ends(const double *pos_dist, uint64_t n_sites, const ngsld_params *p, uint32_t *row_end) try {
  if (p == nullptr || row_end == nullptr || n_sites == 0 || n_sites >= 0xffffffffull) return NGSLD_ERR_INVALID;
  std::vector<double> pd;
  if (pos_dist == nullptr)
    pd.assign(n_sites, std::numeric_limits<double>::infinity());
  else
// ... 12 lines not shown
```

ngsld_amd/csrc/engine_run.hip:

```cpp
#include "engine.h"
#include "../../include/ngsld_host.h"

namespace ngsld {
namespace eng {

hipError_t timed_launch(ngsld_ctx *c, const PairArgs &a, hipStream_t stream) {
  if (c->ev_used == c->ev_pool.size()) {
    hipEvent_t b, e;
    hipError_t r = hipEventCreate(&b);
    if (r != hipSuccess) return r;
    r = hipEventCreate(&e);
    if (r != hipSuccess) return r;
    c->ev_pool.emplace_back(b, e);
  }
  auto &ev = c->ev_pool[c->ev_used++];
  hipError_t r = hipEventRecord(ev.first, stream);
  if (r != hipSuccess) return r;
  r = launch_pair_kernel(c->cfg, c->params.ignore_miss_data != 0, a, stream);
  if (r != hipSuccess) return r;
  return hipEventRecord(ev.second, stream);
}

PairArgs make_args(ngsld_ctx *c, uint64_t r0, uint64_t r1, ngsld_rec_std *d_std, ngsld_rec_ext *d_ext, uint32_t *d_flags,
                   uint32_t flag_cap, uint64_t flag_n) {
  PairArgs a{};
  a.flags = d_flags;
  a.flags_host = d_flags != nullptr ? d_flags + flag_head_words(flag_cap) + flag_bitmap_words(flag_n) : nullptr;
  a.flag_cap = flag_cap;
  a.flag_text = 1;
  a.pearson_on_device = lkl_device_eligible(c) ? 1 : 0;
  a.skip_degenerate = (d_flags != nullptr && c->h_skip_count > 0 && c->skip_on && lkl_device_eligible(c) && !c->exact_failed) ? 1 : 0;
  a.planes = c->d_planes.p;
  a.site_stride = 3ull * c->np;
  a.np = c->np;
  a.n_ind = (uint32_t)c->n_ind;
  a.inv_n = 1.0 / (double)c->n_ind;
  a.maf = c->d_maf.p;
  a.mean_e = c->d_mean.p;
  a.rsx = c->d_rsx.p;
  a.items = c->d_items.p + c->h_item_off[r0];
  a.n_items = c->h_item_off[r1] - c->h_item_off[r0];
  if (uses_runs(c->cfg.kernel)) {
    a.runs = c->d_runs.p + c->h_run_off[r0];
    a.n_runs = c->h_run_off[r1] - c->h_run_off[r0];
  }
  a.hard_masks = c->d_hard_masks.p;
  a.hard_u = c->d_hard_u.p;
  a.mask_words = c->mask_words;
  a.items_all = c->d_items.p;
  a.item_off = c->d_item_off.p;
  a.h_item_off = c->h_item_off.data();
  a.row0 = (uint32_t)r0;
  a.row1 = (uint32_t)r1;
  a.planes_bytes = c->n_sites * 3ull * c->np * sizeof(double);
  a.sc4 = c->d_sc4.p;
  a.out_base = c->h_row_off[r0];
  a.out_std = d_std;
  a.out_ext = d_ext;
  a.status = c->d_status.p;
  return a;
}
}
}

extern "C" {

int ngsld_set_text_output(ngsld_ctx *c, const char *const *labels, int enable) try {
  if (c == nullptr) return NGSLD_ERR_INVALID;
  if (!c->have_geno) return fail(c, NGSLD_ERR_INVALID, "set the genotype data before the labels");
  HIP_TRY(c, hipSetDevice(c->device));
  (void)hipGetLastError();
  c->text_mode = false;
  c->clear_blocks();
  if (!enable) return NGSLD_OK;
  c->have_labels = labels != nullptr;
  c->max_label = 6;
  if (labels != nullptr) {
    std::vector<uint64_t> off(c->n_sites + 1, 0);
    for (uint64_t s = 0; s < c->n_sites; ++s) {
      if (labels[s] == nullptr) return fail(c, NGSLD_ERR_INVALID, "a label is NULL");
      const uint64_t n = std::strlen(labels[s]);
      off[s + 1] = off[s] + n;
      c->max_label = std::max<uint64_t>(c->max_label, n);
    }
    std::vector<char> blob(off[c->n_sites] ? off[c->n_sites] : 1);
    for (uint64_t s = 0; s < c->n_sites; ++s) std::memcpy(blob.data() + off[s], labels[s], off[s + 1] - off[s]);
    HIP_TRY(c, c->d_labels.resize(blob.size()));
    HIP_TRY(c, c->d_label_off.resize(c->n_sites + 1));
    HIP_TRY(c, hipMemcpy(c->d_labels.p, blob.data(), blob.size(), hipMemcpyHostToDevice));
    HIP_TRY(c, hipMemcpy(c->d_label_off.p, off.data(), off.size() * sizeof(uint64_t), hipMemcpyHostToDevice));
  }
  c->text_mode = true;
  return NGSLD_OK;
} NGSLD_CATCH(c)

int ngsld_reserve_text_buffers(ngsld_ctx *c, uint64_t bytes_per_row) try {
  if (c == nullptr) return NGSLD_ERR_INVALID;
  if (c->reserve_thread.joinable()) c->reserve_thread.join();
  if (bytes_per_row == 0) return NGSLD_OK;
  const uint64_t bytes_per_batch = bytes_per_row * std::min<uint64_t>(c->batch_pairs, kTextBatchPairs);
  c->reserve_thread = std::thread([c, bytes_per_batch] {
    if (hipSetDevice(c->device) != hipSuccess) return;
    for (int k = 0; k < ngsld_ctx::kSlots; ++k) (void)c->h_text[k].resize(bytes_per_batch);
  });
  return NGSLD_OK;
} NGSLD_CATCH(c)
int ngsld_run_device(ngsld_ctx *c, uint64_t s1_begin, uint64_t s1_end, void *d_std, void *d_ext, void *hip_stream) try {
  if (c == nullptr) return NGSLD_ERR_INVALID;
  if (!c->planned) return fail(c, NGSLD_ERR_INVALID, "ngsld_plan has not been called");
  if (s1_begin > s1_end || s1_end > c->n_sites) return fail(c, NGSLD_ERR_INVALID, "row range out of bounds");
  if (d_std == nullptr) return fail(c, NGSLD_ERR_INVALID, "d_std is NULL");
  HIP_TRY(c, hipSetDevice(c->device));
  (void)hipGetLastError();
  Range range_("ngsld:run_device (pair kernels)");
  {
    const int rcp = finish_device_run(c);
    if (rcp != NGSLD_OK) return rcp;
  }
  hipStream_t st = hip_stream ? (hipStream_t)hip_stream : c->stream;
  c->ev_used = 0;
  c->timed_stream = st;
  c->timed_overlap = false;
  c->timed_pairs = c->h_row_off[s1_end] - c->h_row_off[s1_begin];
  c->replayed_pairs = 0;
  c->replayed_on_device = 0;
  c->flagged_pairs = 0;
  c->text_rows_patched = 0;
  if (c->replay_on) {
    c->flag_cap_dev = flag_cap_for(c->timed_pairs);
    const int rcf = reset_flags(c, c->d_flags_dev, c->timed_pairs, c->flag_cap_dev, st);
    if (rcf != NGSLD_OK) return rcf;
    HIP_TRY(c, c->h_flags_dev.resize(flag_head_words(c->flag_cap_dev)));
  }
  const uint64_t max_items = 0x7ffffff0ull;
  std::vector<uint64_t> cuts;
  for (uint64_t r0 = s1_begin; r0 < s1_end;) {
    uint64_t r1 = r0 + 1;
    while (r1 < s1_end && c->h_item_off[r1 + 1] - c->h_item_off[r0] <= max_items) ++r1;
// ... 922 lines not shown
```

ngsld_amd/csrc/ld_common.h:

```cpp
#pragma once

#include <hip/hip_runtime.h>
#include <stdint.h>

#include "../../include/ngsld.h"

namespace ngsld {

#ifndef NGSLD_PRIO_S
#define NGSLD_PRIO_S 0
#define NGSLD_PRIO_TREE 3
#define NGSLD_PRIO_R 1
#define NGSLD_PRIO_SERIAL 3
#endif
#ifndef NGSLD_SETPRIO
#define NGSLD_SETPRIO 1
#endif
#ifndef NGSLD_MASK_SLOTS
#define NGSLD_MASK_SLOTS 6
#endif
constexpr int kIterMax = 100;
constexpr double kEpsilon = 1e-5;

constexpr double kHapNoise = 0x1p-49;
constexpr double kRecordTol = 2.5e-10;
constexpr double kReplayFloor = 0x1p-30;
constexpr double kTieMargin = 1e-12;
constexpr double kPearsonCond = 0x1p13;
constexpr double kEpsilonTie = kEpsilon + kTieMargin;
constexpr uint32_t kTieBit = 0x80000000u;
constexpr uint64_t kFlagHostOnly = 1ull << 63, kFlagDone = 1ull << 62, kFlagIndexMask = (1ull << 62) - 1;
constexpr uint32_t kFlagListAt = 8;
constexpr uint32_t kFlagHostCap = 1024;
__host__ __device__ inline uint32_t flag_head_words(uint32_t cap) { return kFlagListAt + 2u * cap + 2u * kFlagHostCap; }

typedef ngsld_item Item;

struct Run {
  uint32_t first_item, n_items;
};
#ifndef NGSLD_RUN_ITEMS
#define NGSLD_RUN_ITEMS 16
#endif
constexpr uint32_t kRunItems = NGSLD_RUN_ITEMS;

struct PairArgs {
  const double *planes;
  uint64_t site_stride;
  uint32_t np;
  uint32_t n_ind;
  double inv_n;
  const double *maf;
  const double *mean_e;
  const double *rsx;
  const Item *items;
  uint64_t n_items;
  const struct Run *runs;
  uint64_t n_runs;
  const Item *items_all;
  const double *sc4;
  uint64_t out_base;
  ngsld_rec_std *out_std;
  ngsld_rec_ext *out_ext;
  int *status;
  const uint64_t *hard_masks;
  const double *hard_u;
  uint32_t mask_words;
  uint32_t *flags;
  uint32_t *flags_host;
  uint32_t flag_cap;
  uint32_t flag_text;
  uint32_t pearson_on_device;
  uint32_t skip_degenerate;
  const uint64_t *item_off;
  const uint64_t *h_item_off;
  uint32_t row0, row1, tile_rows, tile_nk;
  uint64_t planes_bytes;
};

typedef unsigned u32x2 __attribute__((ext_vector_type(2)));

__device__ __forceinline__ double mk_double(unsigned lo, unsigned hi) { return __hiloint2double((int)hi, (int)lo); }

__device__ __forceinline__ double ref_nan(double v) { return v != v ? mk_double(0u, 0xfff80000u) : v; }

__device__ __forceinline__ double uniform(double v) {
  return mk_double((unsigned)__builtin_amdgcn_readfirstlane(__double2loint(v)),
                   (unsigned)__builtin_amdgcn_readfirstlane(__double2hiint(v)));
}

__device__ __forceinline__ double read_lane(double v, int lane) {
  return mk_double((unsigned)__builtin_amdgcn_readlane(__double2loint(v), lane),
                   (unsigned)__builtin_amdgcn_readlane(__double2hiint(v), lane));
}

__device__ __forceinline__ double fold32(double x, double y) {
  u32x2 l = __builtin_amdgcn_permlane32_swap((unsigned)__double2loint(x), (unsigned)__double2loint(y), false, false);
  u32x2 h = __builtin_amdgcn_permlane32_swap((unsigned)__double2hiint(x), (unsigned)__double2hiint(y), false, false);
  return mk_double(l[0], h[0]) + mk_double(l[1], h[1]);
}

__device__ __forceinline__ double fold16(double x, double y) {
  u32x2 l = __builtin_amdgcn_permlane16_swap((unsigned)__double2loint(x), (unsigned)__double2loint(y), false, false);
  u32x2 h = __builtin_amdgcn_permlane16_swap((unsigned)__double2hiint(x), (unsigned)__double2hiint(y), false, false);
  return mk_double(l[0], h[0]) + mk_double(l[1], h[1]);
}

template <int CTRL>
__device__ __forceinline__ double dpp_mov(double v) {
  int lo = __double2loint(v), hi = __double2hiint(v);
  lo = __builtin_amdgcn_update_dpp(0, lo, CTRL, 0xf, 0xf, true);
  hi = __builtin_amdgcn_update_dpp(0, hi, CTRL, 0xf, 0xf, true);
  return __hiloint2double(hi, lo);
}

__device__ __forceinline__ void wave_sum4(double &t0, double &t1, double &t2, double &t3) {
  double z01 = fold32(t0, t1);
  double z23 = fold32(t2, t3);
  double w = fold16(z01, z23);
  w += dpp_mov<0x128>(w);
  w += dpp_mov<0x124>(w);
  w += dpp_mov<0x4E>(w);
  w += dpp_mov<0xB1>(w);
  t0 = read_lane(w, 0);
  t2 = read_lane(w, 16);
  t1 = read_lane(w, 32);
  t3 = read_lane(w, 48);
}

template <int CTRL, int ROW_MASK>
__device__ __forceinline__ double dpp_mov_rows(double v) {
  int lo = __double2loint(v), hi = __double2hiint(v);
  lo = __builtin_amdgcn_update_dpp(0, lo, CTRL, ROW_MASK, 0xf, false);
  hi = __builtin_amdgcn_update_dpp(0, hi, CTRL, ROW_MASK, 0xf, false);
  return __hiloint2double(hi, lo);
}

__device__ __forceinline__ double wave_sum3_rows(double t1, double t2, double t3) {
  double z12 = fold32(t1, t2);
  double w = fold16(z12, t3);
  w += dpp_mov<0x128>(w);
  w += dpp_mov<0x124>(w);
  w += dpp_mov<0x4E>(w);
  w += dpp_mov<0xB1>(w);
  w += dpp_mov_rows<0x143, 0x8>(w);
  return w;
}
__device__ __forceinline__ void wave_sum3(double &t1, double &t2, double &t3) {
  double z12 = fold32(t1, t2);
  double w = fold16(z12, t3);
  w += dpp_mov<0x128>(w);
  w += dpp_mov<0x124>(w);
  w += dpp_mov<0x4E>(w);
  w += dpp_mov<0xB1>(w);
  t1 = read_lane(w, 0);
  t2 = read_lane(w, 32);
  int ulo, uhi;
  asm("; undefined" : "=v"(ulo), "=v"(uhi));
  const int lo = __builtin_amdgcn_update_dpp(ulo, __double2loint(w), 0x143, 0x8, 0xf, false);
  const int hi = __builtin_amdgcn_update_dpp(uhi, __double2hiint(w), 0x143, 0x8, 0xf, false);
// ... 87 lines not shown
```

ngsld_amd/csrc/ld_em.h:

```cpp
#pragma once

#include "ld_common.h"

namespace ngsld {

template <int N>
struct RcpTree {
  static constexpr int L = N / 2;
  static __device__ __forceinline__ double prod(const double *s) {
    return RcpTree<L>::prod(s) * RcpTree<N - L>::prod(s + L);
  }
  static __device__ __forceinline__ void down(const double *s, double inv, double *r) {
    const double pl = RcpTree<L>::prod(s), pr = RcpTree<N - L>::prod(s + L);
    RcpTree<L>::down(s, inv * pr, r);
    RcpTree<N - L>::down(s + L, inv * pl, r + L);
  }
};
template <>
struct RcpTree<1> {
  static __device__ __forceinline__ double prod(const double *s) { return s[0]; }
  static __device__ __forceinline__ void down(const double *, double inv, double *r) { r[0] = inv; }
};

struct PairedTag { static constexpr bool value = true; };
// ... 33 lines not shown
  return reinterpret_cast<const double *>((uintptr_t)(((uint64_t)hi << 32) | lo));
}

template <int SLOTS, bool MASKED, bool ONLY_LAST = false, bool UNCENTRED = false, bool A_GLOBAL = false>
__device__ __forceinline__ void stage_pair(const double *pa, uint32_t npa, uint32_t ia0, const double *pb, uint32_t npb,
                                           uint32_t ib0, uint32_t ind0, uint32_t n_ind, double mean1, double mean2,
                                           double (&P)[SLOTS][9], uint32_t &vbits, double &sxy, bool flip_a = false,
                                           bool flip_b = false, const double (*a_regs)[3] = nullptr, int n_a_regs = 0) {
  vbits = 0;
  sxy = 0.0;
  const double *pa0 = pa + (flip_a ? 2 * npa : 0u), *pa1 = pa + npa, *pa2 = pa + (flip_a ? 0u : 2 * npa);
  const double *pb0 = pb + (flip_b ? 2 * npb : 0u), *pb2 = pb + (flip_b ? 0u : 2 * npb);
  if (A_GLOBAL) {
    pa0 = uniform_ptr(pa0); pa1 = uniform_ptr(pa1); pa2 = uniform_ptr(pa2);
  }
  constexpr bool kByCount = !MASKED && !ONLY_LAST;
  const uint32_t lane_in_wave = ind0 & 63u;
  uint32_t n_full = 0, rem = 0;
  if (kByCount) {
    const uint32_t first = ind0 - lane_in_wave;
    const uint32_t have = n_ind > first ? n_ind - first : 0u;
    n_full = (uint32_t)__builtin_amdgcn_readfirstlane((int)(have >> 6 < (uint32_t)SLOTS ? have >> 6 : (uint32_t)SLOTS));
    rem = (uint32_t)__builtin_amdgcn_readfirstlane((int)(have >> 6 < (uint32_t)SLOTS ? have & 63u : 0u));
    vbits = ((1u << n_full) - 1u) | ((lane_in_wave < rem ? 1u : 0u) << n_full);
  }
#pragma unroll
  for (int j = 0; j < SLOTS; ++j) {
    const uint32_t ia = ia0 + (uint32_t)j * 64, ib = ib0 + (uint32_t)j * 64;
    typedef const __attribute__((address_space(1))) double gdouble_t;
    const bool in_regs = a_regs != nullptr && j < n_a_regs;
    const double a0 = in_regs ? a_regs[j < n_a_regs ? j : 0][0] : (A_GLOBAL ? ((gdouble_t *)pa0)[ia] : pa0[ia]),
                 a1 = in_regs ? a_regs[j < n_a_regs ? j : 0][1] : (A_GLOBAL ? ((gdouble_t *)pa1)[ia] : pa1[ia]),
                 a2 = in_regs ? a_regs[j < n_a_regs ? j : 0][2] : (A_GLOBAL ? ((gdouble_t *)pa2)[ia] : pa2[ia]);
    const double b0 = pb0[ib], b1 = pb[npb + ib], b2 = pb2[ib];
    const bool inb = kByCount ? ((vbits >> j) & 1u) != 0
                              : ((ONLY_LAST && j < SLOTS - 1) ? true : ind0 + (uint32_t)j * 64 < n_ind);
    if (!kByCount) {
      bool ok = inb;
      if (MASKED) ok = inb && !miss_data(a0, a1, a2) && !miss_data(b0, b1, b2);
      vbits |= (ok ? 1u : 0u) << j;
    }
    double z0 = a0, z1 = a1, z2 = a2;
    if (MASKED) {
      const double keep = ((vbits >> j) & 1u) ? 1.0 : 0.0;
      z0 = a0 * keep; z1 = a1 * keep; z2 = a2 * keep;
      P[j][0] = fma(z0, b0, 1.0 - keep);
    } else if (ONLY_LAST && j == SLOTS - 1) {
      P[j][0] = fma(a0, b0, inb ? 0.0 : 1.0);
    } else {
      P[j][0] = a0 * b0;
    }
    P[j][1] = z0 * b1; P[j][2] = z0 * b2;
    P[j][3] = z1 * b0; P[j][4] = z1 * b1; P[j][5] = z1 * b2;
    P[j][6] = z2 * b0; P[j][7] = z2 * b1; P[j][8] = z2 * b2;
    if (UNCENTRED && !MASKED) {
      sxy += fma(4.0, P[j][8], fma(2.0, P[j][5] + P[j][7], P[j][4]));
    } else if (UNCENTRED) {
      sxy = fma(fma(2.0, a2, a1), fma(2.0, b2, b1), sxy);
    } else {
      const double c1 = inb ? fma(2.0, a2, a1) - mean1 : 0.0;
      const double c2 = inb ? fma(2.0, b2, b1) - mean2 : 0.0;
      sxy = fma(c1, c2, sxy);
    }
  }
  if (kByCount) {
#pragma unroll
    for (int j = 0; j < SLOTS; ++j) {
      if (n_full <= (uint32_t)j) {
        const bool keep = n_full == (uint32_t)j && lane_in_wave < rem;
        P[j][0] = keep ? P[j][0] : 1.0;
      }
    }
  }
}

template <int SLOTS>
__device__ __forceinline__ uint32_t count_valid(uint32_t vbits) {
  uint32_t x = 0;
#pragma unroll
  for (int j = 0; j < SLOTS; ++j) x += (uint32_t)__popcll(__ballot((vbits >> j) & 1u));
  return x;
}

template <int SLOTS, int WAVES>
__device__ __forceinline__ uint32_t em_pair(const double (&P)[SLOTS][9], uint32_t vbits, double inv_x, double m1,
                                            double m2, double &f0, double &f1, double &f2, double &f3,
                                            double (*xch)[WAVES][4], int sub, int lane, int *status,
                                            uint32_t *xpar = nullptr) {
  static_assert(WAVES == 1 || WAVES == 2 || WAVES == 4 || WAVES == 8, "em_pair: 1, 2, 4 or 8 wavefronts per pair");
  f0 = (1 - m1) * (1 - m2); f1 = (1 - m1) * m2; f2 = m1 * (1 - m2); f3 = m1 * m2;
  if (m1 < 0 || m1 > 1 || m2 < 0 || m2 > 1) {
    if (lane == 0 && sub == 0) atomicExch(status, (int)NGSLD_ERR_MAF_RANGE);
    f0 = f1 = f2 = f3 = __builtin_nan("");
  }
  asm("" : "+v"(inv_x));
  bool bad = false, tie = false;
  uint32_t n_iter = 0;
  constexpr bool kTree = SLOTS > 1;
  constexpr bool kScaled = WAVES == 1;
  auto em_step = [&](auto tree_tag, auto drop_tag, double &n0, double &n1, double &n2, double &n3) {
    constexpr bool kShared = decltype(tree_tag)::value;
    constexpr bool kDrop = decltype(drop_tag)::value;
    static_assert(!kShared || (kTree && kDrop), "the shared-reciprocal step: several slots, three-value form");
    const double p00 = f0 * f0, p01 = f0 * f1, p02 = f0 * f2, p03 = f0 * f3, p11 = f1 * f1;
    const double p12 = f1 * f2, p13 = f1 * f3, p22 = f2 * f2, p23 = f2 * f3, p33 = f3 * f3;
    const double w1 = p01 + p01, w3 = p02 + p02, w4 = 2.0 * (p03 + p12), w5 = p13 + p13, w7 = p23 + p23;
    double R0 = 0, R1 = 0, R2 = 0, R3 = 0, R4 = 0, R5 = 0, R6 = 0, R7 = 0, R8 = 0;
    if (NGSLD_SETPRIO && kShared) __builtin_amdgcn_s_setprio(NGSLD_PRIO_S);
    auto slot_s = [&](int j) -> double {
      double s = p00 * P[j][0];
      s = fma(w1, P[j][1], s); s = fma(p11, P[j][2], s);
      s = fma(w3, P[j][3], s); s = fma(w4, P[j][4], s); s = fma(w5, P[j][5], s);
      s = fma(p22, P[j][6], s); s = fma(w7, P[j][7], s); s = fma(p33, P[j][8], s);
      return s;
    };
    auto slot_acc = [&](int j, double r) {
      if (!kDrop) R0 = fma(P[j][0], r, R0);
      R1 = fma(P[j][1], r, R1); R2 = fma(P[j][2], r, R2);
      R3 = fma(P[j][3], r, R3); R4 = fma(P[j][4], r, R4); R5 = fma(P[j][5], r, R5);
      R6 = fma(P[j][6], r, R6); R7 = fma(P[j][7], r, R7); R8 = fma(P[j][8], r, R8);
    };
    if constexpr (kShared) {
      double sv[SLOTS], rv[SLOTS];
#pragma unroll
      for (int j = 0; j < SLOTS; ++j) sv[j] = slot_s(j);
      if (NGSLD_SETPRIO) __builtin_amdgcn_s_setprio(NGSLD_PRIO_TREE);
      double inv = rcp_refined(RcpTree<SLOTS>::prod(sv));
      if (kScaled) inv *= inv_x;
      RcpTree<SLOTS>::down(sv, inv, rv);
      if (NGSLD_SETPRIO) __builtin_amdgcn_s_setprio(NGSLD_PRIO_R);
#pragma unroll
      for (int j = 0; j < SLOTS; ++j) slot_acc(j, rv[j]);
      if (NGSLD_SETPRIO) __builtin_amdgcn_s_setprio(NGSLD_PRIO_SERIAL);
    } else {
#pragma unroll
      for (int j = 0; j < SLOTS; ++j) {
        if ((vbits >> j) & 1u) slot_acc(j, rcp_refined(slot_s(j)));
      }
    }
    double t0 = kDrop ? 0.0 : fma(p03, R4, fma(p02, R3, fma(p01, R1, p00 * R0)));
    double t1 = fma(p13, R5, fma(p12, R4, fma(p11, R2, p01 * R1)));
    double t2 = fma(p23, R7, fma(p22, R6, fma(p12, R4, p02 * R3)));
    double t3 = fma(p33, R8, fma(p23, R7, fma(p13, R5, p03 * R4)));
    if (WAVES > 1 && kDrop) {
      const double w = wave_sum3_rows(t1, t2, t3);
      const int par = (int)((*xpar)++ & 1u);
      const int row = lane >> 4;
      const uint32_t base = lds_addr(&xch[par][0][0]);
      if ((lane & 15) == 0 && row != 1)
        lds_post(base + (uint32_t)((row == 0 ? 0 : row - 1) * WAVES + sub) * 8u, w);
      lds_barrier();
      if constexpr (WAVES == 8) {
        double v;
        asm volatile("ds_read_b64 %0, %1\n\ts_waitcnt lgkmcnt(0)" : "=&v"(v) : "v"(base + (uint32_t)(lane & 31) * 8u) : "memory");
        v += dpp_mov<0xB1>(v);
        v += dpp_mov<0x4E>(v);
        v += dpp_mov<0x141>(v);
        t1 = read_lane(v, 0); t2 = read_lane(v, 8); t3 = read_lane(v, 16);
      } else {
        constexpr int kHalf = WAVES > 1 ? WAVES / 2 : 1;
        dbl2 q[3 * kHalf];
        lds_gather<3 * kHalf>(base, q);
        t1 = q[0][0] + q[0][1]; t2 = q[kHalf][0] + q[kHalf][1]; t3 = q[2 * kHalf][0] + q[2 * kHalf][1];
#pragma unroll
        for (int v = 1; v < kHalf; ++v) {
          t1 += q[v][0]; t2 += q[kHalf + v][0]; t3 += q[2 * kHalf + v][0];
          t1 += q[v][1]; t2 += q[kHalf + v][1]; t3 += q[2 * kHalf + v][1];
        }
      }
    } else {
      if (kDrop)
        wave_sum3(t1, t2, t3);
      else
        wave_sum4(t0, t1, t2, t3);
      if (WAVES > 1) {
        const int par = (int)((*xpar)++ & 1u);
        if (lane == 0) {
          xch[par][sub][0] = t0; xch[par][sub][1] = t1; xch[par][sub][2] = t2; xch[par][sub][3] = t3;
        }
        lds_barrier();
        t0 = t1 = t2 = t3 = 0.0;
        for (int w = 0; w < WAVES; ++w) {
          t0 += xch[par][w][0]; t1 += xch[par][w][1]; t2 += xch[par][w][2]; t3 += xch[par][w][3];
        }
      }
    }
    const bool scaled = kShared && kScaled;
    n1 = scaled ? t1 : t1 * inv_x; n2 = scaled ? t2 : t2 * inv_x; n3 = scaled ? t3 : t3 * inv_x;
    n0 = kDrop ? 1.0 - ((n1 + n2) + n3) : t0 * inv_x;
  };
  constexpr double kFullBelow = 0x1p-10;
  bool full = __builtin_amdgcn_ballot_w64(f0 < kFullBelow) != 0;
  bool done = false;
  while (!done && n_iter < (uint32_t)kIterMax) {
    if constexpr (kTree) {
      if (!full) {
        for (; n_iter < (uint32_t)kIterMax; ++n_iter) {
          double n0, n1, n2, n3;
          em_step(PairedTag(), PairedTag(), n0, n1, n2, n3);
          if (__builtin_amdgcn_ballot_w64(!(n1 < 2.0))) break;
          bool conv = false;
          if (__builtin_amdgcn_ballot_w64(fabs(n1 - f1) < kEpsilonTie)) {
            const double eps = fmax(fmax(fabs(n0 - f0), fabs(n1 - f1)), fmax(fabs(n2 - f2), fabs(n3 - f3)));
            conv = __builtin_amdgcn_ballot_w64(eps < kEpsilon) != 0;
            tie |= __builtin_amdgcn_ballot_w64(fabs(eps - kEpsilon) < kTieMargin) != 0;
          }
          f0 = n0; f1 = n1; f2 = n2; f3 = n3;
          if (conv) {
            done = true;
            break;
          }
          if (__builtin_amdgcn_ballot_w64(n0 < kFullBelow)) {
            full = true;
            ++n_iter;
            break;
          }
        }
        if (done || n_iter >= (uint32_t)kIterMax) break;
        if (full) continue;
        if (WAVES > 1) lds_barrier();
      }
    }
    double n0, n1, n2, n3;
    if (WAVES == 1 || full)
      em_step(SingleTag(), SingleTag(), n0, n1, n2, n3);
    else
      em_step(SingleTag(), PairedTag(), n0, n1, n2, n3);
    if (__builtin_amdgcn_ballot_w64(!(n1 < 2.0))) {
      bad = true;
      break;
    }
    const double eps = fmax(fmax(fabs(n0 - f0), fabs(n1 - f1)), fmax(fabs(n2 - f2), fabs(n3 - f3)));
    f0 = n0; f1 = n1; f2 = n2; f3 = n3;
    tie |= __builtin_amdgcn_ballot_w64(fabs(eps - kEpsilon) < kTieMargin) != 0;
    if (__builtin_amdgcn_ballot_w64(eps < kEpsilon)) break;
    ++n_iter;
    if (!full && __builtin_amdgcn_ballot_w64(f0 < kFullBelow)) full = true;
  }
  if (bad) f0 = f1 = f2 = f3 = __builtin_nan("");
  return n_iter | (tie ? kTieBit : 0u);
}

__device__ __forceinline__ bool near_rounding(double v, double d) {
  const double t = fabs(v) * 1e6;
  return fabs((t - floor(t)) - 0.5) < d * 1e6;
}

__device__ __forceinline__ bool near_float_midpoint(double x, double d) {
  const float f = (float)x;
  const double lo = 0.5 * ((double)f + (double)nextafterf(f, -__builtin_inff()));
  const double hi = 0.5 * ((double)f + (double)nextafterf(f, __builtin_inff()));
  return fabs(x - lo) <= d || fabs(x - hi) <= d;
}

__device__ __forceinline__ bool chi2_unsettled(double f0, double f1, double f2, double f3, double dh) {
  const double sA = f0 + f1, sB = f0 + f2;
  if (near_float_midpoint(sA, 2 * dh + 0x1p-53 * fabs(sA)) || near_float_midpoint(sB, 2 * dh + 0x1p-53 * fabs(sB))) return true;
  const float freq_A = (float)sA, freq_B = (float)sB;
  const float exp_hap[4] = {freq_A * freq_B, freq_A * (1 - freq_B), (1 - freq_A) * freq_B, (1 - freq_A) * (1 - freq_B)};
  const double h[4] = {f0, f1, f2, f3};
  float chi2 = 0;
  double err = 0;
  for (int i = 0; i < 4; i++) {
    const double e = (double)exp_hap[i];
    const double d = h[i] - e;
    if (e == 0) {
      if (fabs(h[i]) <= dh) return true;
      return false;
    }
    const double t = d * d / e;
    const double s = (double)chi2 + t;
    const double dd = dh + 0x1p-52 * fabs(d);
    const double ds = err + 2 * ((2 * fabs(d) * dd + dd * dd) / e + 0x1p-51 * t) + 0x1p-52 * fabs(s);
    chi2 = (float)s;
    if (near_float_midpoint(s, ds)) {
      const double up = (double)nextafterf(chi2, __builtin_inff()) - (double)chi2;
// ... 76 lines not shown
```

ngsld_amd/csrc/ld_kernel_run.h:

```cpp
#pragma once

#include "ld_run_pipeline.h"

namespace ngsld {

template <int SLOTS, bool MASKED, bool SKIP = false>
__global__ __launch_bounds__(256, 2) void pair_ld_run_kernel(PairArgs A) {
  constexpr int kSiteBytes = SLOTS * 64 * 3 * 8;
  constexpr int kBuf = kSiteBytes + 32;
  constexpr uint32_t kNp = SLOTS * 64;
  constexpr uint32_t kRing = SLOTS <= 9 ? 32 : 8;
  constexpr int kRingOff = kSiteBytes + 4 * kBuf;
  constexpr int kListOff = kRingOff + 4 * (int)(kRing * sizeof(RunResult));
  __shared__ __attribute__((aligned(16))) char smem[kListOff + sizeof(RunList)];
  static_assert(sizeof(smem) <= 81920, "run kernel: two workgroups per CU need <= 80 KB of LDS each");

  const int lane = threadIdx.x & 63;
  const int wave = __builtin_amdgcn_readfirstlane((int)(threadIdx.x >> 6));
  const Run run = A.runs[blockIdx.x];
  const Item *g_items = A.items_all + run.first_item;
  const uint32_t s1 = g_items[0].s1;
  const double m1 = A.sc4[4 * (uint64_t)s1], mean1 = A.sc4[4 * (uint64_t)s1 + 1], rsx1 = A.sc4[4 * (uint64_t)s1 + 2];
  const bool skip1 = SKIP && A.sc4[4 * (uint64_t)s1 + 3] != 0.0;
  char *lds_a = smem;
  char *lds_b = smem + kSiteBytes + wave * kBuf;
  RunResult *ring = reinterpret_cast<RunResult *>(smem + kRingOff) + wave * kRing;
  RunList *L = reinterpret_cast<RunList *>(smem + kListOff);

  dma_site_to_lds<SLOTS>(A.planes + (uint64_t)s1 * A.site_stride, lds_a, lane, wave, 4);
  build_run_list(L, g_items, run.n_items);
  const uint32_t n_kept = (uint32_t)__builtin_amdgcn_readfirstlane((int)L->base[run.n_items]);
  const uint32_t s2_base = (uint32_t)__builtin_amdgcn_readfirstlane((int)L->items[0].s2_begin);
  const uint64_t rec_base = g_items[0].first_record - A.out_base;

  struct Cand {
    uint32_t s2;
    uint64_t rec;
    bool ok;
  };
  auto claim_next = [&]() -> Cand {
    uint32_t j = 0;
    if (lane == 0) j = atomicAdd(&L->claim, 1u);
    j = (uint32_t)__builtin_amdgcn_readfirstlane((int)j);
    if (j >= n_kept) return Cand{0u, 0ull, false};
    const uint32_t off = (uint32_t)__builtin_amdgcn_readfirstlane((int)L->cand[j]);
    return Cand{s2_base + off, rec_base + j, true};
  };
  auto dma_site = [&](uint32_t s2) {
    dma_site_to_lds<SLOTS>(A.planes + (uint64_t)s2 * A.site_stride, lds_b, lane, 0, 1);
    if (lane < 2)
      __builtin_amdgcn_global_load_lds((glb_void_t *)(reinterpret_cast<const char *>(A.sc4 + 4 * (uint64_t)s2) + lane * 16),
                                       (lds_void_t *)(lds_b + kSiteBytes), 16, 0, 0);
  };
  auto flush = [&](uint32_t n) {
    if ((uint32_t)lane < n) {
      const RunResult r = ring[lane];
      write_pair(A, r.rec, r.f[0], r.f[1], r.f[2], r.f[3], r.sxy, rsx1, r.rsx2, r.x, r.n_iter);
    }
  };

  Cand cur = claim_next();
  if (cur.ok) dma_site(cur.s2);
  uint32_t held = 0;
  while (cur.ok) {
    const Cand nxt = claim_next();
    asm volatile("s_waitcnt vmcnt(0)" ::: "memory");
    const double *sc = reinterpret_cast<const double *>(lds_b + kSiteBytes);
    const double m2 = uniform(sc[0]), mean2 = uniform(sc[1]), rsx2 = uniform(sc[2]);
    const bool skip = SKIP && (skip1 || uniform(sc[3]) != 0.0);
    double P[SLOTS][9];
    uint32_t vbits;
    double sxy;
    const Relabel rl = relabel(m1, m2, mean1, mean2);
    stage_pair<SLOTS, MASKED, !MASKED, true>(reinterpret_cast<const double *>(lds_a), kNp, (uint32_t)lane,
                                             reinterpret_cast<const double *>(lds_b), kNp, (uint32_t)lane, (uint32_t)lane,
                                             A.n_ind, rl.mean1, rl.mean2, P, vbits, sxy, rl.flip1, rl.flip2);
    asm volatile("s_waitcnt lgkmcnt(0)" ::: "memory");
    if (nxt.ok) dma_site(nxt.s2);
    const uint32_t x = MASKED ? count_valid<SLOTS>(vbits) : A.n_ind;
    const double inv_x = MASKED ? 1.0 / (double)x : A.inv_n;
    sxy = fma(-(double)A.n_ind * rl.mean1, rl.mean2, wave_sum1_bcast(sxy));
    double f0, f1, f2, f3;
    uint32_t n_iter = 0;
    if (skip) {
      f0 = f1 = f2 = f3 = __builtin_nan("");
    } else {
      n_iter = em_pair<SLOTS, 1>(P, vbits, inv_x, rl.m1, rl.m2, f0, f1, f2, f3, (double (*)[1][4]) nullptr, 0, lane, A.status);
      unrelabel(rl.flip1, rl.flip2, f0, f1, f2, f3);
    }
    if (lane == 0) {
      RunResult &r = ring[held];
      r.f[0] = f0; r.f[1] = f1; r.f[2] = f2; r.f[3] = f3;
      r.sxy = sxy;
      r.rsx2 = rsx2;
      r.x = x;
      r.n_iter = n_iter;
      r.rec = cur.rec;
    }
    if (++held == kRing) {
      flush(held);
      held = 0;
    }
    cur = nxt;
  }
  flush(held);
}

}
```

ngsld_amd/csrc/ld_pair_w1.hip:

```cpp
#include <cstdlib>

#include <algorithm>
#include <cstring>

#include "ld_kernel_run.h"
#include "ld_kernel_group.h"
#include "ld_kernel_stream.h"
#include "ld_dispatch.h"
#include "knobs.h"

namespace ngsld {

bool pair_config(uint64_t n_ind, PairConfig *cfg, int choice, bool masked) {
  if (n_ind == 0 || n_ind >= 0xffffffc0ull) return false;
  cfg->group = 64;
  cfg->waves = 1;
  cfg->form = 0;
  if (choice == kChooseABMulti || choice == kChooseAuto) {
    for (int w = 2; w <= 8; w *= 2) {
      const uint64_t slots = (n_ind + (uint64_t)w * 64 - 1) / ((uint64_t)w * 64);
      const uint64_t lo = choice == kChooseABMulti ? 9 : (!masked && w == 2 ? 11 : 9);
      const uint64_t hi = choice == kChooseABMulti ? 15 : (masked ? (w == 2 ? 13 : 14) : 15);
      if (slots >= lo && slots <= hi) {
        cfg->kernel = kMulti;
        cfg->form = 1;
        cfg->waves = w;
        cfg->slots = (int)slots;
        cfg->np = (uint32_t)(slots * (uint64_t)w * 64);
        return true;
      }
    }
  }
  if (n_ind > 5120u) {
    cfg->kernel = kStream;
    cfg->waves = choice == kChoosePlainStream ? 4 : 8;
    cfg->slots = 0;
    cfg->np = (uint32_t)((n_ind + 63) / 64 * 64);
    return true;
  }
  const bool g32 = n_ind > 128 && n_ind <= 256 && (((n_ind + 31) / 32) & 1ull);
  if (n_ind <= 128 || g32) {
    cfg->kernel = kGroup;
    cfg->group = n_ind <= 64 ? 8 : (n_ind <= 128 ? 16 : 32);
    cfg->slots = (int)((n_ind + (uint64_t)cfg->group - 1) / (uint64_t)cfg->group);
    cfg->np = (uint32_t)(cfg->slots * cfg->group);
    return true;
  }
  const uint64_t slots1 = (n_ind + 63) / 64;
  const bool want_ab = choice == kChooseAB && n_ind > 512 && n_ind <= 1024;
  if (!want_ab && (n_ind <= 512 || (choice == kChooseAuto && slots1 <= 10))) {
    cfg->kernel = kRun;
    cfg->slots = (int)slots1;
    cfg->np = (uint32_t)(slots1 * 64);
    return true;
  }
  if (want_ab || (choice == kChooseAuto && slots1 <= 15)) {
    cfg->kernel = kRunAB;
    cfg->slots = (int)slots1;
    cfg->np = (uint32_t)(slots1 * 64);
    return true;
  }
  int w = 2;
  while ((n_ind + 64ull * w - 1) / (64ull * w) > 8) w *= 2;
  const uint64_t half = (n_ind + 32ull * w - 1) / (32ull * w);
  if (w >= 4 && (half == 9 || half == 10)) w /= 2;
  cfg->waves = w;
  cfg->slots = (int)((n_ind + 64ull * w - 1) / (64ull * w));
  cfg->np = (uint32_t)(cfg->slots * w * 64);
  cfg->kernel = kMulti;
  return true;
}

template <int G, int SLOTS>
static hipError_t launch_g(bool masked, const PairArgs &a, hipStream_t stream) {
  if (a.n_runs == 0) return hipSuccess;
  if (a.n_runs > 0x7fffffffull) return hipErrorInvalidValue;
  const dim3 grid((unsigned)a.n_runs), block(256);
  if (masked)
    hipLaunchKernelGGL((pair_ld_group_kernel<G, SLOTS, true>), grid, block, 0, stream, a);
  else
    hipLaunchKernelGGL((pair_ld_group_kernel<G, SLOTS, false>), grid, block, 0, stream, a);
  return hipGetLastError();
}

template <int G>
static hipError_t launch_group(int slots, bool masked, const PairArgs &a, hipStream_t stream) {
  switch (slots) {
    case 1: return launch_g<G, 1>(masked, a, stream);
    case 2: return launch_g<G, 2>(masked, a, stream);
    case 3: return launch_g<G, 3>(masked, a, stream);
    case 4: return launch_g<G, 4>(masked, a, stream);
    case 5: return launch_g<G, 5>(masked, a, stream);
    case 6: return launch_g<G, 6>(masked, a, stream);
    case 7: return launch_g<G, 7>(masked, a, stream);
    case 8: return launch_g<G, 8>(masked, a, stream);
    default: return hipErrorInvalidValue;
  }
}

template <int SLOTS>
static hipError_t launch_run(bool masked, const PairArgs &a, hipStream_t stream) {
  if (a.n_runs == 0) return hipSuccess;
  if (a.n_runs > 0x7fffffffull) return hipErrorInvalidValue;
  const dim3 grid((unsigned)a.n_runs), block(256);
  if (a.skip_degenerate && a.flags != nullptr) {
    if (masked)
      hipLaunchKernelGGL((pair_ld_run_kernel<SLOTS, true, true>), grid, block, 0, stream, a);
    else
      hipLaunchKernelGGL((pair_ld_run_kernel<SLOTS, false, true>), grid, block, 0, stream, a);
    return hipGetLastError();
  }
  if (masked) {
    hipLaunchKernelGGL((pair_ld_run_kernel<SLOTS, true>), grid, block, 0, stream, a);
    return hipGetLastError();
  }
  hipLaunchKernelGGL((pair_ld_run_kernel<SLOTS, false>), grid, block, 0, stream, a);
  return hipGetLastError();
}

hipError_t launch_pair_wn(int slots, int waves, bool masked, const PairArgs &a, hipStream_t stream);

static hipError_t launch_pair_chunk(const PairConfig &cfg, bool masked, const PairArgs &a, hipStream_t stream);

hipError_t launch_pair_kernel(const PairConfig &cfg, bool masked, const PairArgs &a, hipStream_t stream) {
  uint64_t max_blocks = 1ull << 22;
  if (const char *e = test_knob("MAX_BLOCKS")) {
    const uint64_t u = std::strtoull(e, nullptr, 10);
    if (u >= 1 && u < max_blocks) max_blocks = u;
  }
  if (cfg.kernel == kMulti && cfg.waves > 1 && a.h_item_off != nullptr && a.item_off != nullptr && a.row1 > a.row0 &&
      !test_knob_is("TILES", "0")) {
    uint64_t longest = 0;
    for (uint32_t r = a.row0; r < a.row1; ++r) longest = std::max<uint64_t>(longest, a.h_item_off[r + 1] - a.h_item_off[r]);
    const uint64_t min_items = 32;
    uint64_t min_bytes = 256ull << 20;
    if (const char *e = test_knob("TILE_MIN_MB")) min_bytes = std::strtoull(e, nullptr, 10) << 20;
    if (longest >= min_items && a.planes_bytes >= min_bytes) {
      const uint32_t kTileRows = 64, kGroupRows = 512;
      for (uint32_t g0 = a.row0; g0 < a.row1; g0 += kGroupRows) {
        const uint32_t g1 = std::min<uint32_t>(a.row1, g0 + kGroupRows);
        uint64_t most = 0;
        for (uint32_t r = g0; r < g1; ++r) most = std::max<uint64_t>(most, a.h_item_off[r + 1] - a.h_item_off[r]);
        if (most == 0) continue;
        PairArgs b = a;
        b.row0 = g0;
        b.row1 = g1;
        b.tile_rows = kTileRows;
        b.tile_nk = (uint32_t)((most + 7) / 8);
        const uint64_t row_blocks = (g1 - g0 + kTileRows - 1) / kTileRows;
        const uint64_t blocks = row_blocks * b.tile_nk * kTileRows * 8ull;
        if (blocks > max_blocks) {
          b.tile_nk = 0;
          const uint64_t first = a.h_item_off[g0], count = a.h_item_off[g1] - first;
          for (uint64_t off = 0; off < count; off += max_blocks) {
            b.items = a.items_all + first + off;
            b.n_items = std::min<uint64_t>(max_blocks, count - off);
            const hipError_t e = launch_pair_chunk(cfg, masked, b, stream);
            if (e != hipSuccess) return e;
          }
          continue;
        }
        b.n_items = blocks;
        const hipError_t e = launch_pair_chunk(cfg, masked, b, stream);
        if (e != hipSuccess) return e;
      }
      return hipSuccess;
    }
  }
  const bool by_runs = uses_runs(cfg.kernel);
  const uint64_t total = by_runs ? a.n_runs : a.n_items;
  for (uint64_t off = 0; off < total; off += max_blocks) {
    PairArgs b = a;
    const uint64_t n = total - off < max_blocks ? total - off : max_blocks;
    if (by_runs) {
      b.runs = a.runs + off;
      b.n_runs = n;
    } else {
      b.items = a.items + off;
      b.n_items = n;
    }
    const hipError_t e = launch_pair_chunk(cfg, masked, b, stream);
    if (e != hipSuccess) return e;
  }
  return hipSuccess;
}

static hipError_t launch_pair_chunk(const PairConfig &cfg, bool masked, const PairArgs &a, hipStream_t stream) {
// ... 40 lines not shown
```

ngsld_amd/csrc/ld_prep.h:

```cpp
#pragma once

#include "ld_common.h"

namespace ngsld {

struct PrepArgs {
  const double *raw;
  uint64_t site0;
  const double *maf_in;
  double *planes;
  uint64_t site_stride;
  uint64_t n_sites;
  uint32_t np, n_ind;
  int log_scale, ignore_miss, normalised_input;
  int text_semantics, call_geno;
  int exact_chain;
  double N_thresh, call_thresh;
  double *maf, *mean_e, *rsx;
  int *status;
  int *odd_missing;
  double missing_canon;
};

hipError_t launch_prep(const PrepArgs &a, hipStream_t stream);
struct ItemArgs {
  const uint32_t *row_end;
  const uint8_t *keep;
  const uint64_t *row_seed;
  const uint64_t *row_off;
  const uint64_t *item_off;
  uint64_t *row_count;
  Item *items;
  uint32_t n_sites, span;
  double rnd_sample;
  int count_only;
};
hipError_t launch_items(const ItemArgs &a, hipStream_t stream);
hipError_t launch_pack_scalars(const double *maf, const double *mean_e, const double *rsx, const uint8_t *skip, double *sc4, uint64_t n,
                               hipStream_t stream);
hipError_t launch_site_skip(const double *planes, uint64_t site_stride, uint32_t np, uint32_t n_ind, int ignore_miss, const double *maf,
                            uint64_t n_sites, uint8_t *skip, uint32_t *count, hipStream_t stream);
hipError_t launch_selftest(const double *in, double *out, hipStream_t stream);

}
```

ngsld_amd/csrc/ld_prep.hip:

```cpp
#include "ld_prep.h"
#include "taus.h"

namespace ngsld {

__device__ __forceinline__ double logsum3(double g0, double g1, double g2) {
  double M = g0;
  M = g1 >= M ? g1 : M;
  M = g2 >= M ? g2 : M;
  if (M == -__builtin_inf()) return -__builtin_inf();
  double sum = 0.0;
  sum += exp(g0 - M);
  sum += exp(g1 - M);
  sum += exp(g2 - M);
  return log(sum) + M;
}

__device__ __forceinline__ double conv_log(double g) {
  g = log(g);
  return g == -__builtin_inf() ? -1e15 : g;
}

__device__ __forceinline__ void call_geno(double &g0, double &g1, double &g2, double N_thresh, double call_thresh) {
  int max_pos = 0;
  double mx = -__builtin_inf();
// ... 308 lines not shown
__global__ __launch_bounds__(256) void site_skip_kernel(const double *__restrict__ planes, uint64_t site_stride, uint32_t np, uint32_t n_ind,
                                                        int ignore_miss, const double *__restrict__ maf, uint64_t n_sites,
                                                        uint8_t *__restrict__ skip, uint32_t *count) {
  const int lane = threadIdx.x & 63, wave = threadIdx.x >> 6;
  for (uint64_t site = (uint64_t)blockIdx.x * 4 + wave; site < n_sites; site += (uint64_t)gridDim.x * 4) {
    const double *pl = planes + site * site_stride;
    const double m_in = maf[site];
    const bool flip = m_in > 0.5;
    double m = flip ? 1.0 - m_in : m_in;
    const double *p0 = pl + (flip ? 2ull * np : 0ull), *p1 = pl + np, *p2 = pl + (flip ? 0ull : 2ull * np);
    constexpr int kRegs = MAXJ > 0 ? MAXJ : 1;
    double a0[kRegs], a1[kRegs], a2[kRegs];
    uint32_t valid = 0, x = 0;
    const uint32_t n_slots = (n_ind + 63) / 64;
    auto is_valid = [&](uint32_t i, double g0, double g1, double g2) {
      return i < n_ind && !(ignore_miss && miss_data(g0, g1, g2));
    };
    if (MAXJ > 0) {
#pragma unroll
      for (int j = 0; j < kRegs; ++j) {
        const uint32_t i = (uint32_t)lane + 64u * (uint32_t)j;
        const bool in = i < n_ind;
        a0[j] = in ? p0[i] : 0.0;
        a1[j] = in ? p1[i] : 0.0;
        a2[j] = in ? p2[i] : 0.0;
        if (is_valid(i, a0[j], a1[j], a2[j])) valid |= 1u << j;
      }
      x = 0;
#pragma unroll
      for (int j = 0; j < kRegs; ++j) x += (uint32_t)__popcll(__ballot((valid >> j) & 1u));
    }
    bool mark = false;
    for (int iter = 0; iter < kIterMax; ++iter) {
      const double w0 = (1 - m) * (1 - m), w1 = 2 * m * (1 - m), w2 = m * m;
      double acc = 0.0;
      uint32_t cnt = 0;
      auto one = [&](double g0, double g1, double g2) {
        const double s = fma(w2, g2, fma(w1, g1, w0 * g0));
        acc = fma(fma(2.0 * w2, g2, w1 * g1), rcp_refined(s), acc);
      };
      if (MAXJ > 0) {
#pragma unroll
        for (int j = 0; j < kRegs; ++j)
          if ((valid >> j) & 1u) one(a0[j], a1[j], a2[j]);
        cnt = x;
      } else {
        for (uint32_t j = 0; j < n_slots; ++j) {
          const uint32_t i = (uint32_t)lane + 64u * j;
          const double g0 = i < n_ind ? p0[i] : 0.0, g1 = i < n_ind ? p1[i] : 0.0, g2 = i < n_ind ? p2[i] : 0.0;
          const bool ok = is_valid(i, g0, g1, g2);
          if (ok) one(g0, g1, g2);
          cnt += (uint32_t)__popcll(__ballot(ok));
        }
      }
      const double mn = wave_sum1(acc) / (2.0 * (double)cnt);
      const bool stop = !(fabs(mn - m) >= kEpsilon);
      m = mn;
      if (stop) {
        mark = m < kSkipBelow;
        break;
      }
    }
    if (lane == 0) {
      skip[site] = mark ? 1 : 0;
      if (mark) atomicAdd(count, 1u);
    }
  }
}

hipError_t launch_site_skip(const double *planes, uint64_t site_stride, uint32_t np, uint32_t n_ind, int ignore_miss, const double *maf,
                            uint64_t n_sites, uint8_t *skip, uint32_t *count, hipStream_t stream) {
  if (n_sites == 0) return hipSuccess;
  const uint64_t wgs = (n_sites + 3) / 4;
  const dim3 grid((unsigned)(wgs < 65536 ? wgs : 65536)), block(256);
  if (np <= 512)
    hipLaunchKernelGGL(site_skip_kernel<8>, grid, block, 0, stream, planes, site_stride, np, n_ind, ignore_miss, maf, n_sites, skip, count);
  else if (np <= 1024)
    hipLaunchKernelGGL(site_skip_kernel<16>, grid, block, 0, stream, planes, site_stride, np, n_ind, ignore_miss, maf, n_sites, skip, count);
  else
    hipLaunchKernelGGL(site_skip_kernel<0>, grid, block, 0, stream, planes, site_stride, np, n_ind, ignore_miss, maf, n_sites, skip, count);
  return hipGetLastError();
}

__global__ void pack_scalars_kernel(const double *maf, const double *mean_e, const double *rsx, const uint8_t *skip, double *sc4, uint64_t n) {
  const uint64_t s = (uint64_t)blockIdx.x * blockDim.x + threadIdx.x;
  if (s >= n) return;
  sc4[4 * s] = maf[s];
  sc4[4 * s + 1] = mean_e[s];
  sc4[4 * s + 2] = rsx[s];
  sc4[4 * s + 3] = (skip != nullptr && skip[s]) ? 1.0 : 0.0;
}

hipError_t launch_pack_scalars(const double *maf, const double *mean_e, const double *rsx, const uint8_t *skip, double *sc4, uint64_t n,
                               hipStream_t stream) {
  if (n == 0) return hipSuccess;
  hipLaunchKernelGGL(pack_scalars_kernel, dim3((unsigned)((n + 255) / 256)), dim3(256), 0, stream, maf, mean_e, rsx, skip, sc4, n);
  return hipGetLastError();
}

__global__ void items_kernel(ItemArgs A) {
  const uint32_t s1 = blockIdx.x * blockDim.x + threadIdx.x;
  if (s1 >= A.n_sites) return;
  const uint32_t end = A.row_end[s1];
  const bool sampling = A.row_seed != nullptr;
  Taus rng;
  if (sampling) rng.set(A.row_seed[s1]);
  uint64_t kept = 0;
  uint64_t k = A.count_only ? 0 : A.item_off[s1];
  const uint64_t base = A.count_only ? 0 : A.row_off[s1];
  for (uint32_t b = s1 + 1; b < end; b += A.span) {
    const uint32_t cnt = end - b < A.span ? end - b : A.span;
    uint64_t mask = 0;
    for (uint32_t c = 0; c < cnt; ++c) {
      if (!A.keep[b + c]) continue;
      if (sampling && rng.uniform() > A.rnd_sample) continue;
      mask |= 1ull << c;
    }
    if (!A.count_only) {
      Item it;
      it.s1 = s1;
      it.s2_begin = b;
      it.count = cnt;
      it.reserved = 0;
      it.mask = mask;
      it.first_record = base + kept;
      A.items[k++] = it;
    }
    kept += (uint64_t)__popcll(mask);
  }
  if (A.count_only) A.row_count[s1] = kept;
}

hipError_t launch_items(const ItemArgs &a, hipStream_t stream) {
  if (a.n_sites == 0) return hipSuccess;
  hipLaunchKernelGGL(items_kernel, dim3((a.n_sites + 255) / 256), dim3(256), 0, stream, a);
  return hipGetLastError();
}

__global__ void selftest_kernel(const double *in, double *out) {
  const int lane = threadIdx.x;
  double t0 = in[lane], t1 = in[64 + lane], t2 = in[128 + lane], t3 = in[192 + lane];
  wave_sum4(t0, t1, t2, t3);
  if (lane == 0) {
    out[0] = t0;
    out[1] = t1;
    out[2] = t2;
    out[3] = t3;
  }
  out[4 + lane] = rcp_refined(in[256 + lane]);
  double u1 = in[lane], u2 = in[64 + lane], u3 = in[128 + lane];
  wave_sum3(u1, u2, u3);
  if (lane == 0) {
    out[68] = u1;
    out[69] = u2;
    out[70] = u3;
  }
}

hipError_t launch_selftest(const double *in, double *out, hipStream_t stream) {
  hipLaunchKernelGGL(selftest_kernel, dim3(1), dim3(64), 0, stream, in, out);
  return hipGetLastError();
}

}
```

Baseline: 201.8 million.

## Pre-scale genotype likelihoods per site to shortcut the first EM step

Adds a per-site preprocessing kernel that divides each individual's genotype likelihoods by their HWE-weighted marginal and stores them with the expected-dosage plane in a new 4-plane layout. The run kernel can then do the first EM iteration from plain slot sums of the scaled products, with no per-individual division, and computes sxy from the stored dosages. Sites with MAF 0 or 1 or an unusable likelihood are marked through the sign bit of the packed scalar and keep the ordinary first step. The cost is extra device memory for a copy a third larger than the planes, a prep kernel, and a separate code path whose first-step rounding may differ slightly.

```diff
diff --git a/include/ngsld.h b/include/ngsld.h
--- a/include/ngsld.h
+++ b/include/ngsld.h
@@ -125,6 +125,7 @@
 int ngsld_last_kernel_time(ngsld_ctx *ctx, double *total_ms, uint64_t *n_launches, uint64_t *n_pairs);
 
 const char *ngsld_pair_kernel(const ngsld_ctx *ctx);
+int ngsld_scaled_layout_info(const ngsld_ctx *ctx, int *in_use, uint64_t *sites_unscaled);
 int ngsld_describe_dispatch(uint64_t n_ind, int ignore_miss_data, char *buf, size_t buf_len);
 
 int ngsld_set_tuning(ngsld_ctx *ctx, uint32_t pairs_per_item, uint64_t batch_pairs);
diff --git a/ngsld_amd/capi.py b/ngsld_amd/capi.py
--- a/ngsld_amd/capi.py
+++ b/ngsld_amd/capi.py
@@ -77,7 +77,7 @@
     "ngsld_set_replay_source", "ngsld_set_replay_matrix", "ngsld_set_replay", "ngsld_replay_stats", "ngsld_finish_device",
     "ngsld_set_exact_store", "ngsld_replay_info",
     "ngsld_plan_parts", "ngsld_run_multi", "ngsld_multi_last_distribution", "ngsld_rccl_selftest",
-    "ngsld_last_kernel_time", "ngsld_pair_kernel", "ngsld_describe_dispatch", "ngsld_set_tuning", "ngsld_selftest", "ngsld_selftest_format",
+    "ngsld_last_kernel_time", "ngsld_pair_kernel", "ngsld_scaled_layout_info", "ngsld_describe_dispatch", "ngsld_set_tuning", "ngsld_selftest", "ngsld_selftest_format",
     "ngsld_selftest_printed", "ngsld_reserve_text_buffers",
     "ngsld_window_ends", "ngsld_plan_slabs", "ngsld_slab_sites_for_budget", "ngsld_sites_for_budget", "ngsld_streamed_replay_info", "ngsld_set_memory_budget", "ngsld_device_memory", "ngsld_run_streamed", "ngsld_run_streamed_text",
     "ngsld_host_read_geno_bin_range",
@@ -211,6 +211,8 @@
             L.ngsld_set_text_output.argtypes = [vp, C.POINTER(C.c_char_p), C.c_int]
         L.ngsld_last_kernel_time.argtypes = [vp, C.POINTER(dbl), C.POINTER(u64), C.POINTER(u64)]
         L.ngsld_set_tuning.argtypes = [vp, C.c_uint32, u64]
+        if hasattr(L, "ngsld_scaled_layout_info"):
+            L.ngsld_scaled_layout_info.argtypes = [vp, C.POINTER(C.c_int), C.POINTER(u64)]
         if hasattr(L, "ngsld_pair_kernel"):
             L.ngsld_pair_kernel.argtypes = [vp]
             L.ngsld_pair_kernel.restype = C.c_char_p
@@ -923,6 +925,11 @@
     def pair_kernel(self) -> str:
         return self._L.ngsld_pair_kernel(self._h).decode()
 
+    def scaled_layout_info(self) -> tuple[bool, int]:
+        on, n = C.c_int(), C.c_uint64()
+        self._check(self._L.ngsld_scaled_layout_info(self._h, C.byref(on), C.byref(n)))
+        return bool(on.value), int(n.value)
+
     def last_kernel_time(self) -> tuple[float, int, int]:
         ms, nl, npairs = C.c_double(), C.c_uint64(), C.c_uint64()
         self._check(self._L.ngsld_last_kernel_time(self._h, C.byref(ms), C.byref(nl), C.byref(npairs)))
diff --git a/ngsld_amd/csrc/cli_main.cpp b/ngsld_amd/csrc/cli_main.cpp
--- a/ngsld_amd/csrc/cli_main.cpp
+++ b/ngsld_amd/csrc/cli_main.cpp
@@ -1202,6 +1202,11 @@
     (void)ngsld_replay_info(ctx, &st);
     fprintf(stderr, "==> %lu of %lu pairs replayed in the reference's operation order (%lu on the device, %lu on host threads)\n",
             (unsigned long)st.pairs_replayed, (unsigned long)n_pairs, (unsigned long)st.pairs_on_device, (unsigned long)st.pairs_on_host);
+    int scaled_on = 0;
+    uint64_t unscaled = 0;
+    if (ngsld_scaled_layout_info(ctx, &scaled_on, &unscaled) == NGSLD_OK && scaled_on)
+      fprintf(stderr, "==> %lu sites take the ordinary first EM step (not scaled: frequency 0 or 1, or an individual without a usable likelihood)\n",
+              (unsigned long)unscaled);
   }
 
   if (pars.verbose >= 1) fprintf(stderr, "==> Freeing memory...\n");
diff --git a/ngsld_amd/csrc/engine.h b/ngsld_amd/csrc/engine.h
--- a/ngsld_amd/csrc/engine.h
+++ b/ngsld_amd/csrc/engine.h
@@ -247,6 +247,10 @@
   uint32_t h_skip_count = 0;
   bool skip_on = true;
   bool skip_kernels = false;
+  DevBuf<double> d_scaled;
+  DevBuf<uint8_t> d_scaled_ok;
+  DevBuf<uint32_t> d_unscaled_count;
+  uint32_t h_unscaled_count = 0;
 
   bool planned = false;
   ngsld_params params{};
@@ -558,6 +562,7 @@
 int device_replay(ngsld_ctx *c, uint32_t *d_flags, uint32_t cap, uint64_t out_base, uint64_t n, ngsld_rec_std *d_std,
                   ngsld_rec_ext *d_ext, hipStream_t st, int slot);
 int finish_device_run(ngsld_ctx *c);
-
-}
-}
+int build_scaled_layout(ngsld_ctx *c);
+
+}
+}
diff --git a/ngsld_amd/csrc/engine.hip b/ngsld_amd/csrc/engine.hip
--- a/ngsld_amd/csrc/engine.hip
+++ b/ngsld_amd/csrc/engine.hip
@@ -164,7 +164,10 @@
   } else {
     c->d_skip.release();
   }
-  HIP_TRY(c, launch_pack_scalars(c->d_maf.p, c->d_mean.p, c->d_rsx.p, c->d_skip.p, c->d_sc4.p, n_sites, c->stream));
+  c->d_scaled.release();
+  c->d_scaled_ok.release();
+  c->h_unscaled_count = 0;
+  HIP_TRY(c, launch_pack_scalars(c->d_maf.p, c->d_mean.p, c->d_rsx.p, c->d_skip.p, nullptr, c->d_sc4.p, n_sites, c->stream));
   int &all_hard = c->h_all_hard;
   all_hard = 0;
   const char *hk = test_knob("HARD_KERNEL");
@@ -201,16 +204,47 @@
   } else {
     c->d_hard_masks.release();
     c->d_hard_u.release();
+    const int rcs = build_scaled_layout(c);
+    if (rcs != NGSLD_OK) return rcs;
+    HIP_TRY(c, hipStreamSynchronize(c->stream));
   }
   c->have_geno = true;
   return NGSLD_OK;
 }
+
+int build_scaled_layout(ngsld_ctx *c) {
+  const PairConfig &cfg = c->cfg;
+  const bool want = cfg.kernel == kRun && cfg.slots >= 4 && cfg.slots <= 8 && !c->gopts.ignore_miss_data && !test_knob_is("SCALED_FIRST", "0");
+  const uint64_t bytes = c->n_sites * 4ull * c->np * sizeof(double);
+  const uint64_t keep_free = c->n_sites * 3ull * c->np * sizeof(double) +
+                             (uint64_t)ngsld_ctx::kSlots * (1ull << 23) * (sizeof(ngsld_rec_std) + sizeof(ngsld_rec_ext)) + (768ull << 20);
+  if (want && c->d_scaled.p == nullptr && room_for(bytes, keep_free + (1ull << 30), keep_free)) {
+    if (c->d_scaled.resize((size_t)c->n_sites * 4 * c->np) != hipSuccess) {
+      (void)hipGetLastError();
+      c->d_scaled.release();
+    }
+  }
+  if (c->d_scaled.p == nullptr) {
+    c->d_scaled_ok.release();
+    c->h_unscaled_count = 0;
+    HIP_TRY(c, launch_pack_scalars(c->d_maf.p, c->d_mean.p, c->d_rsx.p, c->d_skip.p, nullptr, c->d_sc4.p, c->n_sites, c->stream));
+    return NGSLD_OK;
+  }
+  HIP_TRY(c, c->d_scaled_ok.resize(c->n_sites));
+  HIP_TRY(c, c->d_unscaled_count.resize(1));
+  HIP_TRY(c, hipMemsetAsync(c->d_unscaled_count.p, 0, sizeof(uint32_t), c->stream));
+  HIP_TRY(c, launch_scale_sites(c->d_planes.p, 3ull * c->np, c->np, (uint32_t)c->n_ind, c->d_maf.p, c->n_sites, c->d_scaled.p, c->d_scaled_ok.p,
+                                c->d_unscaled_count.p, c->stream));
+  HIP_TRY(c, hipMemcpyAsync(&c->h_unscaled_count, c->d_unscaled_count.p, sizeof(uint32_t), hipMemcpyDeviceToHost, c->stream));
+  HIP_TRY(c, launch_pack_scalars(c->d_maf.p, c->d_mean.p, c->d_rsx.p, c->d_skip.p, c->d_scaled_ok.p, c->d_sc4.p, c->n_sites, c->stream));
+  return NGSLD_OK;
+}
 }
 }
 
 extern "C" {
 
-const char *ngsld_version(void) { return "ngsld-amd 0.9.0 (gfx950; reference ngsLD 1.2.1)"; }
+const char *ngsld_version(void) { return "ngsld-amd 0.10.0 (gfx950; reference ngsLD 1.2.1)"; }
 
 int ngsld_create(int device, ngsld_ctx **out) {
   if (out == nullptr) return NGSLD_ERR_INVALID;
@@ -282,7 +316,7 @@
   (void)hipSetDevice(c->device);
   (void)hipDeviceSynchronize();
   if (c->exact_stream) (void)hipStreamDestroy(c->exact_stream);
-  c->d_planes.release(); c->d_maf.release(); c->d_mean.release(); c->d_rsx.release(); c->d_sc4.release(); c->d_runs.release(); c->d_skip.release(); c->d_skip_count.release();
+  c->d_planes.release(); c->d_maf.release(); c->d_mean.release(); c->d_rsx.release(); c->d_sc4.release(); c->d_scaled.release(); c->d_scaled_ok.release(); c->d_unscaled_count.release(); c->d_runs.release(); c->d_skip.release(); c->d_skip_count.release();
   c->d_hard_masks.release(); c->d_hard_u.release(); c->d_all_hard.release();
   c->d_xplanes.release(); c->d_xmaf.release(); c->d_xT.release(); c->d_xdepth.release(); c->d_xperm.release(); c->h_xstage[0].release(); c->h_xstage[1].release();
   c->lane_scratch_dev.release();
@@ -366,6 +400,14 @@
     case kRunAB: return "ab";
     default: return "";
   }
+}
+
+int ngsld_scaled_layout_info(const ngsld_ctx *c, int *in_use, uint64_t *sites_unscaled) {
+  if (c == nullptr) return NGSLD_ERR_INVALID;
+  const bool on = c->have_geno && c->d_scaled.p != nullptr;
+  if (in_use) *in_use = on ? 1 : 0;
+  if (sites_unscaled) *sites_unscaled = on ? c->h_unscaled_count : 0;
+  return NGSLD_OK;
 }
 
 int ngsld_describe_dispatch(uint64_t n_ind, int ignore_miss_data, char *buf, size_t buf_len) {
diff --git a/ngsld_amd/csrc/engine_plan.hip b/ngsld_amd/csrc/engine_plan.hip
--- a/ngsld_amd/csrc/engine_plan.hip
+++ b/ngsld_amd/csrc/engine_plan.hip
@@ -140,7 +140,8 @@
     }
     if (changed) {
       HIP_TRY(c, hipMemcpy(c->d_maf.p, c->h_maf.data(), n * sizeof(double), hipMemcpyHostToDevice));
-      HIP_TRY(c, launch_pack_scalars(c->d_maf.p, c->d_mean.p, c->d_rsx.p, c->d_skip.p, c->d_sc4.p, n, c->stream));
+      const int rcs = build_scaled_layout(c);
+      if (rcs != NGSLD_OK) return rcs;
     }
   }
   plan_rows(c->h_pos_dist, c->h_maf, *p, n, c->h_row_end);
diff --git a/ngsld_amd/csrc/engine_run.hip b/ngsld_amd/csrc/engine_run.hip
--- a/ngsld_amd/csrc/engine_run.hip
+++ b/ngsld_amd/csrc/engine_run.hip
@@ -54,6 +54,7 @@
   a.row1 = (uint32_t)r1;
   a.planes_bytes = c->n_sites * 3ull * c->np * sizeof(double);
   a.sc4 = c->d_sc4.p;
+  a.scaled = (c->cfg.kernel == kRun && !c->params.ignore_miss_data) ? c->d_scaled.p : nullptr;
   a.out_base = c->h_row_off[r0];
   a.out_std = d_std;
   a.out_ext = d_ext;
diff --git a/ngsld_amd/csrc/ld_common.h b/ngsld_amd/csrc/ld_common.h
--- a/ngsld_amd/csrc/ld_common.h
+++ b/ngsld_amd/csrc/ld_common.h
@@ -76,6 +76,7 @@
   const uint64_t *h_item_off;
   uint32_t row0, row1, tile_rows, tile_nk;
   uint64_t planes_bytes;
+  const double *scaled;
 };
 
 typedef unsigned u32x2 __attribute__((ext_vector_type(2)));
diff --git a/ngsld_amd/csrc/ld_em.h b/ngsld_amd/csrc/ld_em.h
--- a/ngsld_amd/csrc/ld_em.h
+++ b/ngsld_amd/csrc/ld_em.h
@@ -139,11 +139,12 @@
   return x;
 }
 
-template <int SLOTS, int WAVES>
+template <int SLOTS, int WAVES, bool UNIT_FIRST = false>
 __device__ __forceinline__ uint32_t em_pair(const double (&P)[SLOTS][9], uint32_t vbits, double inv_x, double m1,
                                             double m2, double &f0, double &f1, double &f2, double &f3,
                                             double (*xch)[WAVES][4], int sub, int lane, int *status,
-                                            uint32_t *xpar = nullptr) {
+                                            uint32_t *xpar = nullptr, bool unit_first = false) {
+  static_assert(!UNIT_FIRST || (WAVES == 1 && SLOTS > 1), "em_pair: the unit first step is the one-wavefront hot loop's");
   static_assert(WAVES == 1 || WAVES == 2 || WAVES == 4 || WAVES == 8, "em_pair: 1, 2, 4 or 8 wavefronts per pair");
   f0 = (1 - m1) * (1 - m2); f1 = (1 - m1) * m2; f2 = m1 * (1 - m2); f3 = m1 * m2;
   if (m1 < 0 || m1 > 1 || m2 < 0 || m2 > 1) {
@@ -249,6 +250,39 @@
   constexpr double kFullBelow = 0x1p-10;
   bool full = __builtin_amdgcn_ballot_w64(f0 < kFullBelow) != 0;
   bool done = false;
+  if constexpr (UNIT_FIRST) {
+    if (unit_first && !full) {
+      double R1 = 0, R2 = 0, R3 = 0, R4 = 0, R5 = 0, R6 = 0, R7 = 0, R8 = 0;
+#pragma unroll
+      for (int j = 0; j < SLOTS; ++j) {
+        R1 += P[j][1]; R2 += P[j][2]; R3 += P[j][3]; R4 += P[j][4];
+        R5 += P[j][5]; R6 += P[j][6]; R7 += P[j][7]; R8 += P[j][8];
+      }
+      const double p01 = f0 * f1, p02 = f0 * f2, p03 = f0 * f3, p11 = f1 * f1, p12 = f1 * f2;
+      const double p13 = f1 * f3, p22 = f2 * f2, p23 = f2 * f3, p33 = f3 * f3;
+      double t1 = fma(p13, R5, fma(p12, R4, fma(p11, R2, p01 * R1)));
+      double t2 = fma(p23, R7, fma(p22, R6, fma(p12, R4, p02 * R3)));
+      double t3 = fma(p33, R8, fma(p23, R7, fma(p13, R5, p03 * R4)));
+      wave_sum3(t1, t2, t3);
+      const double n1 = t1 * inv_x, n2 = t2 * inv_x, n3 = t3 * inv_x;
+      const double n0 = 1.0 - ((n1 + n2) + n3);
+      if (!__builtin_amdgcn_ballot_w64(!(n1 < 2.0))) {
+        bool conv = false;
+        if (__builtin_amdgcn_ballot_w64(fabs(n1 - f1) < kEpsilonTie)) {
+          const double eps = fmax(fmax(fabs(n0 - f0), fabs(n1 - f1)), fmax(fabs(n2 - f2), fabs(n3 - f3)));
+          conv = __builtin_amdgcn_ballot_w64(eps < kEpsilon) != 0;
+          tie |= __builtin_amdgcn_ballot_w64(fabs(eps - kEpsilon) < kTieMargin) != 0;
+        }
+        f0 = n0; f1 = n1; f2 = n2; f3 = n3;
+        if (conv) {
+          done = true;
+        } else {
+          n_iter = 1;
+          full = __builtin_amdgcn_ballot_w64(n0 < kFullBelow) != 0;
+        }
+      }
+    }
+  }
   while (!done && n_iter < (uint32_t)kIterMax) {
     if constexpr (kTree) {
       if (!full) {
diff --git a/ngsld_amd/csrc/ld_kernel_run.h b/ngsld_amd/csrc/ld_kernel_run.h
--- a/ngsld_amd/csrc/ld_kernel_run.h
+++ b/ngsld_amd/csrc/ld_kernel_run.h
@@ -4,8 +4,9 @@
 
 namespace ngsld {
 
-template <int SLOTS, bool MASKED, bool SKIP = false>
+template <int SLOTS, bool MASKED, bool SKIP = false, bool SCALED = false>
 __global__ __launch_bounds__(256, 2) void pair_ld_run_kernel(PairArgs A) {
+  static_assert(!SCALED || (!MASKED && SLOTS >= 4 && SLOTS <= 8), "run kernel: the scaled layout is the unmasked four-to-eight-slot shapes'");
   constexpr int kSiteBytes = SLOTS * 64 * 3 * 8;
   constexpr int kBuf = kSiteBytes + 32;
   constexpr uint32_t kNp = SLOTS * 64;
@@ -21,13 +22,17 @@
   const Item *g_items = A.items_all + run.first_item;
   const uint32_t s1 = g_items[0].s1;
   const double m1 = A.sc4[4 * (uint64_t)s1], mean1 = A.sc4[4 * (uint64_t)s1 + 1], rsx1 = A.sc4[4 * (uint64_t)s1 + 2];
-  const bool skip1 = SKIP && A.sc4[4 * (uint64_t)s1 + 3] != 0.0;
+  const double mark1 = A.sc4[4 * (uint64_t)s1 + 3];
+  const bool skip1 = SKIP && mark1 != 0.0;
+  const bool unit1 = SCALED && __builtin_signbit(mark1);
+  const double *sites = SCALED ? A.scaled : A.planes;
+  const uint64_t site_stride = SCALED ? 4ull * kNp : A.site_stride;
   char *lds_a = smem;
   char *lds_b = smem + kSiteBytes + wave * kBuf;
   RunResult *ring = reinterpret_cast<RunResult *>(smem + kRingOff) + wave * kRing;
   RunList *L = reinterpret_cast<RunList *>(smem + kListOff);
 
-  dma_site_to_lds<SLOTS>(A.planes + (uint64_t)s1 * A.site_stride, lds_a, lane, wave, 4);
+  dma_site_to_lds<SLOTS>(sites + (uint64_t)s1 * site_stride, lds_a, lane, wave, 4);
   build_run_list(L, g_items, run.n_items);
   const uint32_t n_kept = (uint32_t)__builtin_amdgcn_readfirstlane((int)L->base[run.n_items]);
   const uint32_t s2_base = (uint32_t)__builtin_amdgcn_readfirstlane((int)L->items[0].s2_begin);
@@ -47,7 +52,7 @@
     return Cand{s2_base + off, rec_base + j, true};
   };
   auto dma_site = [&](uint32_t s2) {
-    dma_site_to_lds<SLOTS>(A.planes + (uint64_t)s2 * A.site_stride, lds_b, lane, 0, 1);
+    dma_site_to_lds<SLOTS>(sites + (uint64_t)s2 * site_stride, lds_b, lane, 0, 1);
     if (lane < 2)
       __builtin_amdgcn_global_load_lds((glb_void_t *)(reinterpret_cast<const char *>(A.sc4 + 4 * (uint64_t)s2) + lane * 16),
                                        (lds_void_t *)(lds_b + kSiteBytes), 16, 0, 0);
@@ -63,11 +68,30 @@
   if (cur.ok) dma_site(cur.s2);
   uint32_t held = 0;
   while (cur.ok) {
+    double e1[SLOTS], e2[SLOTS];
+    if (SCALED) {
+      typedef const __attribute__((address_space(1))) double gdouble_t;
+      gdouble_t *g1 = (gdouble_t *)(sites + (uint64_t)s1 * site_stride + 3u * kNp + (uint32_t)lane);
+      gdouble_t *g2 = (gdouble_t *)(sites + (uint64_t)cur.s2 * site_stride + 3u * kNp + (uint32_t)lane);
+#pragma unroll
+      for (int j = 0; j < SLOTS; ++j) {
+        e1[j] = g1[64 * j];
+        e2[j] = g2[64 * j];
+      }
+    }
     const Cand nxt = claim_next();
     asm volatile("s_waitcnt vmcnt(0)" ::: "memory");
+    double sxy_e = 0.0;
+    if (SCALED) {
+#pragma unroll
+      for (int j = 0; j < SLOTS; ++j) sxy_e = fma(e1[j], e2[j], sxy_e);
+      asm volatile("" : "+v"(sxy_e));
+    }
     const double *sc = reinterpret_cast<const double *>(lds_b + kSiteBytes);
     const double m2 = uniform(sc[0]), mean2 = uniform(sc[1]), rsx2 = uniform(sc[2]);
-    const bool skip = SKIP && (skip1 || uniform(sc[3]) != 0.0);
+    const double mark2 = uniform(sc[3]);
+    const bool skip = SKIP && (skip1 || mark2 != 0.0);
+    const bool unit = SCALED && unit1 && __builtin_signbit(mark2);
     double P[SLOTS][9];
     uint32_t vbits;
     double sxy;
@@ -79,13 +103,18 @@
     if (nxt.ok) dma_site(nxt.s2);
     const uint32_t x = MASKED ? count_valid<SLOTS>(vbits) : A.n_ind;
     const double inv_x = MASKED ? 1.0 / (double)x : A.inv_n;
-    sxy = fma(-(double)A.n_ind * rl.mean1, rl.mean2, wave_sum1_bcast(sxy));
+    sxy = SCALED ? fma(-(double)A.n_ind * mean1, mean2, wave_sum1_bcast(sxy_e))
+                 : fma(-(double)A.n_ind * rl.mean1, rl.mean2, wave_sum1_bcast(sxy));
     double f0, f1, f2, f3;
     uint32_t n_iter = 0;
     if (skip) {
       f0 = f1 = f2 = f3 = __builtin_nan("");
     } else {
-      n_iter = em_pair<SLOTS, 1>(P, vbits, inv_x, rl.m1, rl.m2, f0, f1, f2, f3, (double (*)[1][4]) nullptr, 0, lane, A.status);
+      if constexpr (SCALED)
+        n_iter = em_pair<SLOTS, 1, true>(P, vbits, inv_x, rl.m1, rl.m2, f0, f1, f2, f3, (double (*)[1][4]) nullptr, 0, lane, A.status, nullptr,
+                                         unit);
+      else
+        n_iter = em_pair<SLOTS, 1>(P, vbits, inv_x, rl.m1, rl.m2, f0, f1, f2, f3, (double (*)[1][4]) nullptr, 0, lane, A.status);
       unrelabel(rl.flip1, rl.flip2, f0, f1, f2, f3);
     }
     if (lane == 0) {
diff --git a/ngsld_amd/csrc/ld_pair_w1.hip b/ngsld_amd/csrc/ld_pair_w1.hip
--- a/ngsld_amd/csrc/ld_pair_w1.hip
+++ b/ngsld_amd/csrc/ld_pair_w1.hip
@@ -103,6 +103,16 @@
   if (a.n_runs == 0) return hipSuccess;
   if (a.n_runs > 0x7fffffffull) return hipErrorInvalidValue;
   const dim3 grid((unsigned)a.n_runs), block(256);
+  if constexpr (SLOTS >= 4 && SLOTS <= 8) {
+    if (!masked && a.scaled != nullptr) {
+      if (a.np != (uint32_t)SLOTS * 64u) return hipErrorInvalidValue;
+      if (a.skip_degenerate && a.flags != nullptr)
+        hipLaunchKernelGGL((pair_ld_run_kernel<SLOTS, false, true, true>), grid, block, 0, stream, a);
+      else
+        hipLaunchKernelGGL((pair_ld_run_kernel<SLOTS, false, false, true>), grid, block, 0, stream, a);
+      return hipGetLastError();
+    }
+  }
   if (a.skip_degenerate && a.flags != nullptr) {
     if (masked)
       hipLaunchKernelGGL((pair_ld_run_kernel<SLOTS, true, true>), grid, block, 0, stream, a);
diff --git a/ngsld_amd/csrc/ld_prep.h b/ngsld_amd/csrc/ld_prep.h
--- a/ngsld_amd/csrc/ld_prep.h
+++ b/ngsld_amd/csrc/ld_prep.h
@@ -36,8 +36,10 @@
   int count_only;
 };
 hipError_t launch_items(const ItemArgs &a, hipStream_t stream);
-hipError_t launch_pack_scalars(const double *maf, const double *mean_e, const double *rsx, const uint8_t *skip, double *sc4, uint64_t n,
-                               hipStream_t stream);
+hipError_t launch_pack_scalars(const double *maf, const double *mean_e, const double *rsx, const uint8_t *skip, const uint8_t *scaled_ok,
+                               double *sc4, uint64_t n, hipStream_t stream);
+hipError_t launch_scale_sites(const double *planes, uint64_t site_stride, uint32_t np, uint32_t n_ind, const double *maf, uint64_t n_sites,
+                              double *scaled, uint8_t *ok, uint32_t *n_unscaled, hipStream_t stream);
 hipError_t launch_site_skip(const double *planes, uint64_t site_stride, uint32_t np, uint32_t n_ind, int ignore_miss, const double *maf,
                             uint64_t n_sites, uint8_t *skip, uint32_t *count, hipStream_t stream);
 hipError_t launch_selftest(const double *in, double *out, hipStream_t stream);
diff --git a/ngsld_amd/csrc/ld_prep.hip b/ngsld_amd/csrc/ld_prep.hip
--- a/ngsld_amd/csrc/ld_prep.hip
+++ b/ngsld_amd/csrc/ld_prep.hip
@@ -414,19 +414,72 @@
   return hipGetLastError();
 }
 
-__global__ void pack_scalars_kernel(const double *maf, const double *mean_e, const double *rsx, const uint8_t *skip, double *sc4, uint64_t n) {
+__global__ __launch_bounds__(256) void scale_sites_kernel(const double *__restrict__ planes, uint64_t site_stride, uint32_t np, uint32_t n_ind,
+                                                          const double *__restrict__ maf, uint64_t n_sites, double *__restrict__ scaled,
+                                                          uint8_t *__restrict__ ok, uint32_t *n_unscaled) {
+  const int lane = threadIdx.x & 63, wave = threadIdx.x >> 6;
+  for (uint64_t site = (uint64_t)blockIdx.x * 4 + wave; site < n_sites; site += (uint64_t)gridDim.x * 4) {
+    const double *pl = planes + site * site_stride;
+    double *out = scaled + site * 4ull * np;
+    const double m_in = maf[site];
+    const bool flip = m_in > 0.5;
+    const double m = flip ? 1.0 - m_in : m_in;
+    const double u0 = (1 - m) * (1 - m), u1 = 2 * m * (1 - m), u2 = m * m;
+    const double *p0 = pl + (flip ? 2ull * np : 0ull), *p1 = pl + np, *p2 = pl + (flip ? 0ull : 2ull * np);
+    bool good = m_in > 0.0 && m_in < 1.0;
+    for (uint32_t i = (uint32_t)lane; i < n_ind; i += 64) {
+      const double a0 = p0[i], a1 = p1[i], a2 = p2[i];
+      const double d = fma(u2, a2, fma(u1, a1, u0 * a0));
+      const double top = fmax(a0, fmax(a1, a2)) / d;
+      good = good && !odd_triple(a0, a1, a2) && d > 0.0 && d < __builtin_inf() && top < __builtin_inf();
+    }
+    good = __ballot(!good) == 0;
+    for (uint32_t i = (uint32_t)lane; i < np; i += 64) {
+      double a0 = 0.0, a1 = 0.0, a2 = 0.0, e = 0.0;
+      if (i < n_ind) {
+        a0 = pl[i]; a1 = pl[np + i]; a2 = pl[2ull * np + i];
+        e = fma(2.0, a2, a1);
+        if (good) {
+          const double d = flip ? fma(u2, a0, fma(u1, a1, u0 * a2)) : fma(u2, a2, fma(u1, a1, u0 * a0));
+          a0 /= d; a1 /= d; a2 /= d;
+        }
+      }
+      out[i] = a0;
+      out[np + i] = a1;
+      out[2ull * np + i] = a2;
+      out[3ull * np + i] = e;
+    }
+    if (lane == 0) {
+      ok[site] = good ? 1 : 0;
+      if (!good) atomicAdd(n_unscaled, 1u);
+    }
+  }
+}
+
+hipError_t launch_scale_sites(const double *planes, uint64_t site_stride, uint32_t np, uint32_t n_ind, const double *maf, uint64_t n_sites,
+                              double *scaled, uint8_t *ok, uint32_t *n_unscaled, hipStream_t stream) {
+  if (n_sites == 0) return hipSuccess;
+  const uint64_t wgs = (n_sites + 3) / 4;
+  hipLaunchKernelGGL(scale_sites_kernel, dim3((unsigned)(wgs < 65536 ? wgs : 65536)), dim3(256), 0, stream, planes, site_stride, np, n_ind, maf,
+                     n_sites, scaled, ok, n_unscaled);
+  return hipGetLastError();
+}
+
+__global__ void pack_scalars_kernel(const double *maf, const double *mean_e, const double *rsx, const uint8_t *skip, const uint8_t *scaled_ok,
+                                    double *sc4, uint64_t n) {
   const uint64_t s = (uint64_t)blockIdx.x * blockDim.x + threadIdx.x;
   if (s >= n) return;
   sc4[4 * s] = maf[s];
   sc4[4 * s + 1] = mean_e[s];
   sc4[4 * s + 2] = rsx[s];
-  sc4[4 * s + 3] = (skip != nullptr && skip[s]) ? 1.0 : 0.0;
-}
-
-hipError_t launch_pack_scalars(const double *maf, const double *mean_e, const double *rsx, const uint8_t *skip, double *sc4, uint64_t n,
-                               hipStream_t stream) {
+  const double mark = (skip != nullptr && skip[s]) ? 1.0 : 0.0;
+  sc4[4 * s + 3] = (scaled_ok != nullptr && scaled_ok[s]) ? -mark : mark;
+}
+
+hipError_t launch_pack_scalars(const double *maf, const double *mean_e, const double *rsx, const uint8_t *skip, const uint8_t *scaled_ok,
+                               double *sc4, uint64_t n, hipStream_t stream) {
   if (n == 0) return hipSuccess;
-  hipLaunchKernelGGL(pack_scalars_kernel, dim3((unsigned)((n + 255) / 256)), dim3(256), 0, stream, maf, mean_e, rsx, skip, sc4, n);
+  hipLaunchKernelGGL(pack_scalars_kernel, dim3((unsigned)((n + 255) / 256)), dim3(256), 0, stream, maf, mean_e, rsx, skip, scaled_ok, sc4, n);
   return hipGetLastError();
 }
 
```

Result: no change. 202.5 million (median of 6 runs) (+0.3%).
